# MattAgostini/ECE1782-Smith-Waterman-CUDA

Measured on AMD Instinct MI355X. Metric: GCUPS (DP cell updates/s) query-vs-SwissProt, 1/2/4/8 MI355X; bit-exact scores, higher is better.
Workload: dtype fp16

## Files before the change

ece1782-smith-waterman-cuda_amd/capi.py:

```python
import ctypes
import os
import weakref

import numpy as np

PKG_DIR = os.path.dirname(os.path.abspath(__file__))
LIB_DIR = os.path.join(PKG_DIR, "lib")
LIB_PATH = os.environ.get("SW_AMD_LIB") or os.path.join(LIB_DIR, "libswamd.so")

SW_OK = 0
SW_ALPHABET = 25
MATRIX_BLOSUM50_REF = 0
MATRIX_BLOSUM62 = 1
MATRIX_IDENTITY3 = 2
MATRIX_BLOSUM50_CHAR = 3

EXPORTED = (
    "sw_version", "sw_build_id", "sw_last_error", "sw_encode", "sw_builtin_matrix",
    "sw_create", "sw_destroy", "sw_stream", "sw_set_stream",
    "sw_opts_init", "sw_opts_from_env", "sw_set_opts", "sw_get_opts",
    "sw_db_create", "sw_db_free", "sw_db_get_stats", "sw_db_set_long_threshold", "sw_db_reset_adaptive",
    "sw_scan", "sw_scan_device", "sw_scan_batch", "sw_scan_batch_device", "sw_get_timing",
    "sw_timing_reset", "sw_timing_total", "sw_stream_wait_scan", "sw_last_kernel", "sw_last_intra_kernel",
    "sw_topk", "sw_topk_device", "sw_topk_keys_device", "sw_topk_device_ids", "sw_scan_topk",
    "sw_scan_rank_device", "sw_score_pair",
    "sw_align",
    "sw_pssm_create", "sw_pssm_free", "sw_pssm_length", "sw_scan_pssm", "sw_scan_pssm_device",
    "sw_scan_pssm_topk", "sw_align_pssm",
    "sw_db_save", "sw_db_load", "sw_db_subjects", "sw_db_create_synthetic", "sw_synth_tables",
    "sw_synth_lengths", "sw_group_create", "sw_group_destroy", "sw_group_info", "sw_group_handle",
    "sw_group_db_create", "sw_group_db_free", "sw_group_db_shard", "sw_group_scan", "sw_group_topk",
)


class SWError(RuntimeError):
    pass


class Scoring(ctypes.Structure):
    _fields_ = [("matrix", ctypes.POINTER(ctypes.c_int8)),
                ("gap_open", ctypes.c_int32),
                ("gap_extend", ctypes.c_int32)]


class DbStats(ctypes.Structure):
    _fields_ = [("n_subjects", ctypes.c_int64), ("residues", ctypes.c_int64),
                ("packed_cells", ctypes.c_int64), ("n_blocks", ctypes.c_int64),
                ("n_long", ctypes.c_int64), ("device_bytes", ctypes.c_int64),
                ("max_length", ctypes.c_int32), ("long_threshold", ctypes.c_int32),
                ("coop_blocks", ctypes.c_int32), ("coop_residues", ctypes.c_int64),
                ("max_id", ctypes.c_int32), ("pair_blocks", ctypes.c_int32),
                ("pair_merged", ctypes.c_int32), ("pair_residues", ctypes.c_int64)]


class Alignment(ctypes.Structure):
    _fields_ = [("score", ctypes.c_int32), ("q_begin", ctypes.c_int32), ("q_end", ctypes.c_int32),
                ("s_begin", ctypes.c_int32), ("s_end", ctypes.c_int32), ("ops_len", ctypes.c_int32)]


class Opts(ctypes.Structure):
    INT_FIELDS = ("lpt", "lpt_pipe", "quad_width", "pair_width", "pair_group", "coop_width", "coop_skew",
                  "intra_x2", "intra_x2_rows", "intra_i16_first", "inter_i16_span", "int16_guard",
                  "rescue_stats", "tail_pairs", "lpt_persist", "lpt_rows", "tri_width", "lpt_pipe_tail", "drain_spin")
    _fields_ = [("size", ctypes.c_int32)] + [(f, ctypes.c_int32) for f in INT_FIELDS] + \
        [("inter_variant", ctypes.c_char * 16), ("trace_file", ctypes.c_char * 256)]

    def as_dict(self):
        d = {f: getattr(self, f) for f in self.INT_FIELDS}
        d["inter_variant"] = self.inter_variant.decode()
        d["trace_file"] = self.trace_file.decode()
        return d


def opts_from_env():
    o = Opts()
    _check(lib().sw_opts_from_env(ctypes.byref(o)))
    return o


class Timing(ctypes.Structure):
    _fields_ = [("inter_ms", ctypes.c_float), ("intra_ms", ctypes.c_float),
                ("total_ms", ctypes.c_float), ("rescued", ctypes.c_int32),
                ("launches", ctypes.c_int32), ("coop_ms", ctypes.c_float),
                ("wave_ms", ctypes.c_float)]


_LIB = None


def lib():
    global _LIB
    if _LIB is not None:
        return _LIB
    if not os.path.exists(LIB_PATH):
        raise SWError("HIP library %s not built; run __graft_entry__.build() "
                      "or make -C ece1782-smith-waterman-cuda_amd/csrc" % LIB_PATH)
    try:
        import torch
    except ImportError:
        pass
    L = ctypes.CDLL(LIB_PATH)
    vp, i32, i64 = ctypes.c_void_p, ctypes.c_int32, ctypes.c_int64
    u8p = ctypes.POINTER(ctypes.c_uint8)
    i32p = ctypes.POINTER(ctypes.c_int32)
    i64p = ctypes.POINTER(ctypes.c_int64)
    sig = {
        "sw_version": (i32, []),
        "sw_build_id": (ctypes.c_char_p, []),
        "sw_last_error": (ctypes.c_char_p, []),
        "sw_encode": (ctypes.c_int, [ctypes.c_char_p, i64, u8p]),
        "sw_builtin_matrix": (ctypes.c_int, [i32, ctypes.POINTER(ctypes.c_int8)]),
        "sw_create": (ctypes.c_int, [i32, ctypes.POINTER(vp)]),
        "sw_destroy": (ctypes.c_int, [vp]),
        "sw_stream": (vp, [vp]),
        "sw_set_stream": (ctypes.c_int, [vp, vp]),
        "sw_opts_init": (ctypes.c_int, [ctypes.POINTER(Opts)]),
        "sw_opts_from_env": (ctypes.c_int, [ctypes.POINTER(Opts)]),
        "sw_set_opts": (ctypes.c_int, [vp, ctypes.POINTER(Opts)]),
        "sw_get_opts": (ctypes.c_int, [vp, ctypes.POINTER(Opts)]),
        "sw_db_reset_adaptive": (ctypes.c_int, [vp]),
        "sw_db_create": (ctypes.c_int, [vp, u8p, i64p, i64, i32p, ctypes.POINTER(vp)]),
        "sw_db_free": (ctypes.c_int, [vp]),
        "sw_db_get_stats": (ctypes.c_int, [vp, ctypes.POINTER(DbStats)]),
        "sw_db_set_long_threshold": (ctypes.c_int, [vp, i32]),
        "sw_scan": (ctypes.c_int, [vp, vp, u8p, i32, ctypes.POINTER(Scoring), i32p]),
        "sw_scan_device": (ctypes.c_int, [vp, vp, u8p, i32, ctypes.POINTER(Scoring), vp]),
        "sw_scan_batch": (ctypes.c_int, [vp, vp, u8p, i64p, i32, ctypes.POINTER(Scoring), i32p]),
        "sw_scan_batch_device": (ctypes.c_int, [vp, vp, u8p, i64p, i32, ctypes.POINTER(Scoring), vp]),
        "sw_get_timing": (ctypes.c_int, [vp, ctypes.POINTER(Timing)]),
        "sw_timing_reset": (ctypes.c_int, [vp]),
        "sw_timing_total": (ctypes.c_int, [vp, ctypes.POINTER(Timing), i32p]),
        "sw_stream_wait_scan": (ctypes.c_int, [vp, vp]),
        "sw_last_kernel": (ctypes.c_char_p, [vp]),
        "sw_last_intra_kernel": (ctypes.c_char_p, [vp]),
        "sw_db_save": (ctypes.c_int, [vp, ctypes.c_char_p]),
        "sw_db_create_synthetic": (ctypes.c_int, [vp, ctypes.c_uint64, i64, i64, ctypes.POINTER(vp)]),
        "sw_synth_tables": (ctypes.c_int, [i32p, u8p]),
        "sw_synth_lengths": (ctypes.c_int, [ctypes.c_uint64, i64, i64, i32p]),
        "sw_db_subjects": (ctypes.c_int, [vp, i64p, i32p]),
        "sw_db_load": (ctypes.c_int, [vp, ctypes.c_char_p, ctypes.POINTER(vp)]),
        "sw_align": (ctypes.c_int, [vp, vp, u8p, i32, ctypes.POINTER(Scoring), i32p, i32,
                                    ctypes.POINTER(Alignment), ctypes.c_char_p, ctypes.c_int64]),
        "sw_pssm_create": (ctypes.c_int, [vp, ctypes.POINTER(ctypes.c_int8), i32, ctypes.POINTER(vp)]),
        "sw_pssm_free": (ctypes.c_int, [vp]),
        "sw_pssm_length": (ctypes.c_int, [vp, i32p]),
        "sw_scan_pssm": (ctypes.c_int, [vp, vp, vp, i32, i32, i32p]),
        "sw_scan_pssm_device": (ctypes.c_int, [vp, vp, vp, i32, i32, vp]),
        "sw_scan_pssm_topk": (ctypes.c_int, [vp, vp, vp, i32, i32, i32, i64p]),
        "sw_align_pssm": (ctypes.c_int, [vp, vp, vp, i32, i32, i32p, i32,
                                         ctypes.POINTER(Alignment), ctypes.c_char_p, ctypes.c_int64]),
        "sw_topk": (ctypes.c_int, [i32p, i64, i32, i32p, i32p]),
        "sw_topk_device": (ctypes.c_int, [vp, vp, i64, i64, i32, vp]),
        "sw_topk_keys_device": (ctypes.c_int, [vp, vp, i64, i32, vp]),
        "sw_topk_device_ids": (ctypes.c_int, [vp, vp, i64, vp, i32, vp]),
        "sw_scan_topk": (ctypes.c_int, [vp, vp, u8p, i32, ctypes.POINTER(Scoring), i32, i64p]),
        "sw_scan_rank_device": (ctypes.c_int, [vp, vp, u8p, i32, ctypes.POINTER(Scoring), vp, i32, vp, i64, vp]),
        "sw_score_pair": (ctypes.c_int, [vp, u8p, i32, u8p, i32, ctypes.POINTER(Scoring), i32p]),
        "sw_group_create": (ctypes.c_int, [i32p, i32, ctypes.POINTER(vp)]),
        "sw_group_destroy": (ctypes.c_int, [vp]),
        "sw_group_info": (ctypes.c_char_p, [vp]),
        "sw_group_handle": (ctypes.c_int, [vp, i32, ctypes.POINTER(vp)]),
        "sw_group_db_create": (ctypes.c_int, [vp, u8p, i64p, i64, i32p, ctypes.POINTER(vp)]),
        "sw_group_db_free": (ctypes.c_int, [vp]),
        "sw_group_db_shard": (ctypes.c_int, [vp, i32, i64p, i64p]),
        "sw_group_scan": (ctypes.c_int, [vp, vp, u8p, i32, ctypes.POINTER(Scoring), i32p]),
        "sw_group_topk": (ctypes.c_int, [vp, vp, u8p, i32, ctypes.POINTER(Scoring), i32, i64p]),
    }
    for name, (res, args) in sig.items():
        fn = getattr(L, name)
        fn.restype = res
        fn.argtypes = args
    built, want = L.sw_build_id().decode(), source_id()
    if built != want:
        raise SWError("stale HIP library %s: built from sources %s, the tree's are %s; rebuild it "
                      "(__graft_entry__.build() or make -C ece1782-smith-waterman-cuda_amd/csrc)"
                      % (LIB_PATH, built, want))
    _LIB = L
    return L


def source_id(repo_root=None):
    import importlib.util
    spec = importlib.util.spec_from_file_location("_sw_build_id", os.path.join(PKG_DIR, "csrc", "build_id.py"))
    mod = importlib.util.module_from_spec(spec)
    spec.loader.exec_module(mod)
    return mod.source_id(repo_root or os.path.dirname(PKG_DIR))


def build_id():
    return lib().sw_build_id().decode()


def _check(rc):
    if rc != SW_OK:
        raise SWError("sw_amd error %d: %s" % (rc, lib().sw_last_error().decode(errors="replace")))


def _u8(a):
    a = np.ascontiguousarray(a, dtype=np.uint8)
    return a, a.ctypes.data_as(ctypes.POINTER(ctypes.c_uint8))


def encode(seq):
    b = seq.encode() if isinstance(seq, str) else bytes(seq)
    out = np.empty(len(b), dtype=np.uint8)
    _check(lib().sw_encode(b, len(b), out.ctypes.data_as(ctypes.POINTER(ctypes.c_uint8))))
    return out


def builtin_matrix(mid=MATRIX_BLOSUM50_REF):
    out = np.empty(625, dtype=np.int8)
    _check(lib().sw_builtin_matrix(mid, out.ctypes.data_as(ctypes.POINTER(ctypes.c_int8))))
    return out.reshape(25, 25)


class _ScoringArg:

    def __init__(self, matrix=None, gap_open=2, gap_extend=None):
        gap_extend = gap_open if gap_extend is None else gap_extend
        if matrix is None:
            self._m = None
            self.s = Scoring(None, gap_open, gap_extend)
        else:
            self._m = np.ascontiguousarray(np.asarray(matrix, dtype=np.int8).reshape(625))
            self.s = Scoring(self._m.ctypes.data_as(ctypes.POINTER(ctypes.c_int8)), gap_open, gap_extend)

    def ptr(self):
        return ctypes.byref(self.s)


class Handle:

    def __init__(self, device=0, env_opts=True):
        h = ctypes.c_void_p()
        _check(lib().sw_create(device, ctypes.byref(h)))
        self._h = h
        self.device = device
        self._dbs = weakref.WeakSet()
        if env_opts:
            _check(lib().sw_set_opts(h, ctypes.byref(opts_from_env())))

    def get_opts(self):
        o = Opts()
        _check(lib().sw_get_opts(self._h, ctypes.byref(o)))
        return o

    def set_opts(self, opts=None, **fields):
        o = Opts()
        if opts is None:
            o = self.get_opts()
        else:
            ctypes.memmove(ctypes.byref(o), ctypes.byref(opts), ctypes.sizeof(Opts))
        for k, v in fields.items():
            if k in ("inter_variant", "trace_file"):
                setattr(o, k, (v or "").encode())
            elif k in Opts.INT_FIELDS:
                setattr(o, k, -1 if v is None else int(v))
            else:
                raise TypeError("unknown sw_opts field %r" % k)
        _check(lib().sw_set_opts(self._h, ctypes.byref(o)))

    def reset_opts(self):
        o = Opts()
        _check(lib().sw_opts_init(ctypes.byref(o)))
        _check(lib().sw_set_opts(self._h, ctypes.byref(o)))

    @property
    def ptr(self):
        return self._h

    def close(self):
        if self._h:
            for db in list(self._dbs):
                db.close()
            lib().sw_destroy(self._h)
            self._h = None

    def __del__(self):
        try:
            self.close()
        except Exception:
            pass

    def stream(self):
        return lib().sw_stream(self._h)

    def set_stream(self, hip_stream):
        _check(lib().sw_set_stream(self._h, hip_stream))

    def timing(self):
        t = Timing()
        _check(lib().sw_get_timing(self._h, ctypes.byref(t)))
        return {k: getattr(t, k) for k, _ in Timing._fields_}

    def timing_reset(self):
        _check(lib().sw_timing_reset(self._h))

    def stream_wait_scan(self, hip_stream):
        _check(lib().sw_stream_wait_scan(self._h, hip_stream))

    def last_kernel(self):
        return lib().sw_last_kernel(self._h).decode()

    def last_intra_kernel(self):
        return lib().sw_last_intra_kernel(self._h).decode()

    def timing_total(self):
        t = Timing()
        n = ctypes.c_int32()
        _check(lib().sw_timing_total(self._h, ctypes.byref(t), ctypes.byref(n)))
        out = {k: getattr(t, k) for k, _ in Timing._fields_ if k != "rescued"}
        out["scans"] = n.value
        return out

    def topk_device(self, scores_dev_ptr, n, k, keys_out_dev_ptr, id_base=0):
        _check(lib().sw_topk_device(self._h, ctypes.c_void_p(scores_dev_ptr), n, id_base, k,
                                    ctypes.c_void_p(keys_out_dev_ptr)))

    def topk_device_ids(self, scores_dev_ptr, n, ids_dev_ptr, k, keys_out_dev_ptr):
        _check(lib().sw_topk_device_ids(self._h, ctypes.c_void_p(scores_dev_ptr), n, ctypes.c_void_p(ids_dev_ptr),
                                        k, ctypes.c_void_p(keys_out_dev_ptr)))

    def topk_keys_device(self, keys_dev_ptr, n, k, keys_out_dev_ptr):
        _check(lib().sw_topk_keys_device(self._h, ctypes.c_void_p(keys_dev_ptr), n, k,
                                         ctypes.c_void_p(keys_out_dev_ptr)))

    def score_pair(self, query_codes, subject_codes, matrix=None, gap_open=2, gap_extend=None):
        q, qp = _u8(query_codes)
        s, sp = _u8(subject_codes)
        sc = _ScoringArg(matrix, gap_open, gap_extend)
        out = ctypes.c_int32()
        _check(lib().sw_score_pair(self._h, qp, len(q), sp, len(s), sc.ptr(), ctypes.byref(out)))
        return out.value


class Pssm:

    def __init__(self, handle, rows):
        self.handle = handle
        r = np.asarray(rows)
        if r.size and (r.ndim != 2 or r.shape[1] != SW_ALPHABET):
            raise SWError("a PSSM is a [qlen][%d] table" % SW_ALPHABET)
        if r.size and (r.min() < -128 or r.max() > 127):
            raise SWError("sw_amd error -1: PSSM entries must be in -100..100")
        r = np.ascontiguousarray(r, dtype=np.int8).reshape(-1, SW_ALPHABET)
        p = ctypes.c_void_p()
        _check(lib().sw_pssm_create(handle.ptr, r.ctypes.data_as(ctypes.POINTER(ctypes.c_int8)), len(r),
                                    ctypes.byref(p)))
        self._p = p
        handle._dbs.add(self)

    @property
    def ptr(self):
        return self._p

    def __len__(self):
        n = ctypes.c_int32()
        _check(lib().sw_pssm_length(self._p, ctypes.byref(n)))
        return n.value

    def close(self):
        if self._p:
            if self.handle.ptr:
                lib().sw_pssm_free(self._p)
            self._p = None

    def __del__(self):
        try:
            self.close()
        except Exception:
            pass


class Database:

    def __init__(self, handle, residues, offsets, ids=None, long_threshold=None):
        self.handle = handle
        r, rp = _u8(residues)
        o = np.ascontiguousarray(offsets, dtype=np.int64)
        n = len(o) - 1
        idp = None
        if ids is not None:
            self._ids = np.ascontiguousarray(ids, dtype=np.int32)
            idp = self._ids.ctypes.data_as(ctypes.POINTER(ctypes.c_int32))
            self.n_out = int(self._ids.max()) + 1 if n > 0 else 0
        else:
            self.n_out = n
        d = ctypes.c_void_p()
        _check(lib().sw_db_create(handle.ptr, rp, o.ctypes.data_as(ctypes.POINTER(ctypes.c_int64)),
                                  n, idp, ctypes.byref(d)))
        self._d = d
        self.n = n
        handle._dbs.add(self)
        if long_threshold is not None:
            self.set_long_threshold(long_threshold)

    @classmethod
    def synthetic(cls, handle, seed, n, id_base=0, long_threshold=None):
        self = cls.__new__(cls)
        self.handle = handle
        d = ctypes.c_void_p()
        _check(lib().sw_db_create_synthetic(handle.ptr, seed, id_base, n, ctypes.byref(d)))
        self._d = d
        self.n = n
        self.n_out = n
        handle._dbs.add(self)
        if long_threshold is not None:
            self.set_long_threshold(long_threshold)
        return self
# ... 265 lines not shown
```

ece1782-smith-waterman-cuda_amd/csrc/sw_capi.cpp:

```cpp
#include <algorithm>
#include <cmath>
#include <atomic>
#include <cstdio>
#include <cstdlib>
#include <cstring>
#include <memory>
#include <new>
#include <numeric>
#include <string>
#include <thread>
#include <unordered_map>
#include <vector>

#include "sw_host.h"
#include "sw_plan.h"

using swk::DevPtr;
using swk::Event;
using swk::HostPtr;
using swk::Stream;

namespace {

thread_local std::string g_err;

constexpr int kF16Span = 2048;

uint32_t f16_pair(int v) {
    const _Float16 x = static_cast<_Float16>(static_cast<float>(v));
    uint16_t b;
    std::memcpy(&b, &x, 2);
    return static_cast<uint32_t>(b) | (static_cast<uint32_t>(b) << 16);
}

int fail(int code, const std::string& msg) {
    g_err = msg;
    return code;
}

#define MARK(k, s)                                  \
    do {                                            \
        HIPCHECK(hipEventRecord(h->ev[k].get(), (s)));    \
        *h->ev_rec |= 1u << (k);                    \
    } while (0)

const int8_t kBlosum50Ref[625] = {
    5, -2, -1, -2, -1, -1, -1, 0, -2, -1, -2, -1, -1, -3, -1, 1, 0, -3, -2, 0, -2, -2, -1, -1, 0,
    -2, 7, -1, -2, -4, 1, 0, -3, 0, -4, -3, 3, -2, -3, -3, -1, -1, -3, -1, -3, -1, -3, 0, -1, 0,
    -1, -1, 7, 2, -2, 0, 0, 0, 1, -3, -4, 0, -2, -4, -2, 1, 0, -4, -2, -3, 5, -4, 0, -1, 0,
    -2, -2, 2, 8, -4, 0, 2, -1, -1, -4, -4, -1, -4, -5, -1, 0, -1, -5, -3, -4, 6, -4, 1, -1, 0,
    -1, -4, -2, -4, 13, -3, -3, -3, -3, -2, -2, -3, -2, -2, -4, -1, -1, -5, -3, -1, -3, -2, -3, -1, 0,
    -1, 1, 0, 0, -3, 7, 2, -2, 1, -3, -2, 2, 0, -4, -1, 0, -1, -1, -1, -3, 0, -3, 4, -1, 0,
    -1, 0, 0, 2, -3, 2, 6, -3, 0, -4, -3, 1, -2, -3, -1, -1, -1, -3, -2, -3, 1, -3, 5, -1, 0,
    0, -3, 0, -1, -3, -2, -3, 8, -2, -4, -4, -2, -3, -4, -2, 0, -2, -3, -3, -4, -1, -4, -2, -1, 0,
    -2, 0, 1, -1, -3, 1, 0, -2, 10, -4, -3, 0, -1, -1, -2, -1, -2, -3, 2, -4, 0, -3, 0, -1, 0,
    -1, -4, -3, -4, -2, -3, -4, -4, -4, 5, 2, -3, 2, 0, -3, -3, -1, -3, -1, 4, -4, 4, -3, -1, 0,
    -2, -3, -4, -4, -2, -2, -3, -4, -3, 2, 5, -3, 3, 1, -4, -3, -1, -2, -1, 1, -4, 4, -3, -1, 0,
    -1, 3, 0, -1, -3, 2, 1, -2, 0, -3, -3, 6, -2, -4, -1, 0, -1, -3, -2, -3, 0, -3, 1, -1, 0,
    -1, -2, -2, -4, -2, 0, -2, -3, -1, 2, 3, -2, 7, 0, -3, -2, -1, -1, 0, 1, -3, 2, -1, -1, 0,
    -3, -3, -4, -5, -2, -4, -3, -4, -1, 0, 1, -4, 0, 8, -4, -3, -2, 1, 4, -1, -4, 1, -4, -1, 0,
    -1, -3, -2, -1, -4, -1, -1, -2, -2, -3, -4, -1, -3, -4, 10, -1, -1, -4, -3, -3, -2, -3, -1, -1, 0,
    1, -1, 1, 0, -1, 0, -1, 0, -1, -3, -3, 0, -2, -3, -1, 5, 2, -4, -2, -2, 0, -3, 0, -1, 0,
    0, -1, 0, -1, -1, -1, -1, -2, -2, -1, -1, -1, -1, -2, -1, 2, 5, -3, -2, 0, 0, -1, -1, -1, 0,
    -3, -3, -4, -5, -5, -1, -3, -3, -3, -3, -2, -3, -1, 1, -4, -4, -3, 15, 2, -3, -5, -2, -2, -1, 0,
    -2, -1, -2, -3, -3, -1, -2, -3, 2, -1, -1, -2, 0, 4, -3, -2, -2, 2, 8, -1, -3, -1, -2, -1, 0,
    0, -3, -3, -4, -1, -3, -3, -4, -4, 4, 1, -3, 1, -1, -3, -2, 0, -3, -1, 5, -3, 2, -3, -1, 0,
    -2, -1, 5, 6, -3, 0, 1, -1, 0, -4, -4, 0, -3, -4, -2, 0, 0, -5, -3, -3, 6, -4, 1, -1, 0,
    -2, -3, -4, -4, -2, -3, -3, -4, -3, 4, 4, -3, 2, 1, -3, -3, -1, -2, -1, 2, -4, 4, -3, -1, 0,
    -1, 0, 0, 1, -3, 4, 5, -2, 0, -3, -3, 1, -1, -4, -1, 0, -1, -2, -2, -3, 1, -3, 5, -1, 0,
    -1, -1, -1, -1, -1, -1, -1, -1, -1, -1, -1, -1, -1, -1, -1, -1, -1, -1, -1, -1, -1, -1, -1, -1, 0,
    0, 0, 0, 0, 0, 0, 0, 0, 0, 0, 0, 0, 0, 0, 0, 0, 0, 0, 0, 0, 0, 0, 0, 0, 0,
};

const int8_t kBlosum62[625] = {
    4, -1, -2, -2, 0, -1, -1, 0, -2, -1, -1, -1, -1, -2, -1, 1, 0, -3, -2, 0, -2, -1, -1, 0, -4,
    -1, 5, 0, -2, -3, 1, 0, -2, 0, -3, -2, 2, -1, -3, -2, -1, -1, -3, -2, -3, -1, -2, 0, -1, -4,
    -2, 0, 6, 1, -3, 0, 0, 0, 1, -3, -3, 0, -2, -3, -2, 1, 0, -4, -2, -3, 3, -3, 0, -1, -4,
    -2, -2, 1, 6, -3, 0, 2, -1, -1, -3, -4, -1, -3, -3, -1, 0, -1, -4, -3, -3, 4, -3, 1, -1, -4,
    0, -3, -3, -3, 9, -3, -4, -3, -3, -1, -1, -3, -1, -2, -3, -1, -1, -2, -2, -1, -3, -1, -3, -2, -4,
    -1, 1, 0, 0, -3, 5, 2, -2, 0, -3, -2, 1, 0, -3, -1, 0, -1, -2, -1, -2, 0, -2, 3, -1, -4,
    -1, 0, 0, 2, -4, 2, 5, -2, 0, -3, -3, 1, -2, -3, -1, 0, -1, -3, -2, -2, 1, -3, 4, -1, -4,
    0, -2, 0, -1, -3, -2, -2, 6, -2, -4, -4, -2, -3, -3, -2, 0, -2, -2, -3, -3, -1, -4, -2, -1, -4,
    -2, 0, 1, -1, -3, 0, 0, -2, 8, -3, -3, -1, -2, -1, -2, -1, -2, -2, 2, -3, 0, -3, 0, -1, -4,
    -1, -3, -3, -3, -1, -3, -3, -4, -3, 4, 2, -3, 1, 0, -3, -2, -1, -3, -1, 3, -3, 3, -3, -1, -4,
    -1, -2, -3, -4, -1, -2, -3, -4, -3, 2, 4, -2, 2, 0, -3, -2, -1, -2, -1, 1, -4, 3, -3, -1, -4,
    -1, 2, 0, -1, -3, 1, 1, -2, -1, -3, -2, 5, -1, -3, -1, 0, -1, -3, -2, -2, 0, -3, 1, -1, -4,
    -1, -1, -2, -3, -1, 0, -2, -3, -2, 1, 2, -1, 5, 0, -2, -1, -1, -1, -1, 1, -3, 2, -1, -1, -4,
    -2, -3, -3, -3, -2, -3, -3, -3, -1, 0, 0, -3, 0, 6, -4, -2, -2, 1, 3, -1, -3, 0, -3, -1, -4,
    -1, -2, -2, -1, -3, -1, -1, -2, -2, -3, -3, -1, -2, -4, 7, -1, -1, -4, -3, -2, -2, -3, -1, -2, -4,
    1, -1, 1, 0, -1, 0, 0, 0, -1, -2, -2, 0, -1, -2, -1, 4, 1, -3, -2, -2, 0, -2, 0, 0, -4,
    0, -1, 0, -1, -1, -1, -1, -2, -2, -1, -1, -1, -1, -2, -1, 1, 5, -2, -2, 0, -1, -1, -1, 0, -4,
    -3, -3, -4, -4, -2, -2, -3, -2, -2, -3, -2, -3, -1, 1, -4, -3, -2, 11, 2, -3, -4, -2, -3, -2, -4,
    -2, -2, -2, -3, -2, -1, -2, -3, 2, -1, -1, -2, -1, 3, -3, -2, -2, 2, 7, -1, -3, -1, -2, -1, -4,
    0, -3, -3, -3, -1, -2, -2, -3, -3, 3, 1, -2, 1, -1, -2, -2, 0, -3, -1, 4, -3, 2, -2, -1, -4,
    -2, -1, 3, 4, -3, 0, 1, -1, 0, -3, -4, 0, -3, -3, -2, 0, -1, -4, -3, -3, 4, -3, 1, -1, -4,
    -1, -2, -3, -3, -1, -2, -3, -4, -3, 3, 3, -3, 2, 0, -3, -2, -1, -2, -1, 2, -3, 3, -3, -1, -4,
    -1, 0, 0, 1, -3, 3, 4, -2, 0, -3, -3, 1, -1, -3, -1, 0, -1, -3, -2, -2, 1, -3, 4, -1, -4,
    0, -1, -1, -1, -2, -1, -1, -1, -1, -1, -1, -1, -1, -1, -2, 0, 0, -2, -1, -1, -1, -1, -1, -1, -4,
    -4, -4, -4, -4, -4, -4, -4, -4, -4, -4, -4, -4, -4, -4, -4, -4, -4, -4, -4, -4, -4, -4, -4, -4, 1,
};

int8_t g_encode_lut[256];
bool g_lut_ready = false;

void init_lut() {
    if (g_lut_ready) return;
    static const char letters[] = "ARNDCQEGHILKMFPSTWYVBJZX";
    for (int c = 0; c < 256; ++c) g_encode_lut[c] = SW_CODE_STAR;
    for (int k = 0; k < 24; ++k) g_encode_lut[static_cast<unsigned char>(letters[k])] = static_cast<int8_t>(k);
    g_lut_ready = true;
}

int64_t round_up(int64_t v, int64_t m) { return (v + m - 1) / m * m; }

int default_threads() {
    unsigned n = std::thread::hardware_concurrency();
    if (n == 0) n = 4;
    return static_cast<int>(std::min(16u, n));
}

template <class F>
void parallel_for(int64_t n, F&& f, int64_t grain = 64) {
    const int nt = static_cast<int>(std::min<int64_t>(default_threads(), std::max<int64_t>(1, n / grain)));
    if (nt <= 1) {
        for (int64_t i = 0; i < n; ++i) f(i);
        return;
    }
    std::atomic<int64_t> next{0};
    std::vector<std::thread> th;
    for (int t = 0; t < nt; ++t)
        th.emplace_back([&] {
            for (;;) {
                const int64_t i0 = next.fetch_add(grain);
                if (i0 >= n) break;
                const int64_t i1 = std::min(n, i0 + grain);
                for (int64_t i = i0; i < i1; ++i) f(i);
            }
        });
    for (auto& t : th) t.join();
}

template <class T>
struct NoInitAlloc : std::allocator<T> {
    template <class U>
    struct rebind {
        using other = NoInitAlloc<U>;
    };
    NoInitAlloc() = default;
    template <class U>
    NoInitAlloc(const NoInitAlloc<U>&) {}
    template <class U, class... A>
    void construct(U* p, A&&... a) {
        if constexpr (sizeof...(A) == 0) ::new (static_cast<void*>(p)) U;
        else ::new (static_cast<void*>(p)) U(std::forward<A>(a)...);
    }
};

std::vector<int64_t> length_order(const std::vector<int64_t>& offs, int64_t n) {
    std::vector<int64_t> order(n);
    int64_t maxl = 0;
    for (int64_t k = 0; k < n; ++k) maxl = std::max(maxl, offs[k + 1] - offs[k]);
    if (maxl > (int64_t(1) << 22)) {
        std::iota(order.begin(), order.end(), 0);
        std::stable_sort(order.begin(), order.end(), [&](int64_t x, int64_t y) {
            return offs[x + 1] - offs[x] > offs[y + 1] - offs[y];
        });
        return order;
    }
    std::vector<int64_t> start(static_cast<size_t>(maxl) + 2, 0);
    for (int64_t k = 0; k < n; ++k) ++start[static_cast<size_t>(maxl - (offs[k + 1] - offs[k]) + 1)];
    for (size_t l = 1; l < start.size(); ++l) start[l] += start[l - 1];
    for (int64_t k = 0; k < n; ++k) order[start[static_cast<size_t>(maxl - (offs[k + 1] - offs[k]))]++] = k;
    return order;
}

}

int swk::set_error(int code, const std::string& msg) { return fail(code, msg); }

struct ScanEvents {
    Event ev[8];
    unsigned rec = 0;
    int launches = 0;
    bool merged = false;
};

namespace {
sw_opts default_opts() {
    sw_opts o;
    std::memset(&o, 0, sizeof o);
    o.size = static_cast<int32_t>(sizeof o);
    for (int32_t* f : {&o.lpt, &o.lpt_pipe, &o.quad_width, &o.pair_width, &o.pair_group, &o.coop_width,
                       &o.coop_skew, &o.intra_x2, &o.intra_x2_rows, &o.intra_i16_first, &o.inter_i16_span,
                       &o.int16_guard, &o.rescue_stats, &o.tail_pairs, &o.lpt_persist, &o.lpt_rows,
                       &o.tri_width, &o.lpt_pipe_tail, &o.drain_spin})
        *f = -1;
    return o;
}
}

struct sw_handle {
    int device = 0;
    int cus = 0;
    Stream stream;
    bool own_stream = false;
    ~sw_handle() { if (!own_stream) stream.release(); }
    std::vector<ScanEvents> evpool;
    size_t nscans = 0;
    Event* ev = nullptr;
    unsigned* ev_rec = nullptr;
    Stream side;
    Stream side2;
    Stream tail;
    Event main_done, side_done;
    Event tail_done[2];
    bool tail_pending[2] = {};
    int parity = 0;
    Event coop_done;
    Event fork2;
    struct ProfSlot {
        DevPtr<int8_t> d;
        size_t dcap = 0;
        hipEvent_t last_end = nullptr;
        bool pending = false;
        Event tail_read;
        bool tail_pending = false;
    };
    HostPtr<uint8_t> stage[2];
    size_t stage_cap = 0;
    Event stage_ev[2];
    bool stage_pending[2] = {};
    static constexpr int kProfSlots = 4;
    ProfSlot prof[kProfSlots];
    int prof_next = 0;
    DevPtr<int32_t> d_scores;
    size_t scores_cap = 0;
    DevPtr<int64_t> d_topk_work;
    std::string last_kernel = "none";
    std::string last_intra = "none";
    size_t topk_cap = 0;
    bool timed = false;
    bool had_intra = false;
    int launches = 0;
    HostPtr<int32_t> h_fault;
    int32_t* d_fault = nullptr;
    int open_slot = -1;
    sw_opts opts = default_opts();
};

static std::atomic<uint64_t> g_fault_epoch{0};

static int check_fault(sw_handle* h) {
    if (h && h->h_fault.get() && __atomic_load_n(h->h_fault.get(), __ATOMIC_ACQUIRE)) {
        __atomic_store_n(h->h_fault.get(), 0, __ATOMIC_RELEASE);
        g_fault_epoch.fetch_add(1);
        return fail(SW_E_DEVICE, "sw_scan_lpt: a claimed rescue-list entry never appeared; the handle's scans "
                                 "since the last successful call may hold unrescued scores");
    }
    return SW_OK;
}

static hipError_t quiesce(sw_handle* h) {
    hipError_t first = hipSuccess;
    for (hipStream_t st : {h->stream.get(), h->side.get(), h->side2.get(), h->tail.get()})
        if (st) {
            const hipError_t e = hipStreamSynchronize(st);
            if (first == hipSuccess) first = e;
        }
    return first;
}

struct Readback {
    struct Obs {
        uint64_t key = 0, qhash = 0;
        int32_t qlen = 0, nr = 0;
        bool operator==(const Obs& o) const { return key == o.key && qhash == o.qhash && qlen == o.qlen && nr == o.nr; }
    };
    HostPtr<int32_t> host;
    Event ev;
    bool pending = false;
    bool seen = false;
    Obs sent, last;
};

namespace {
int readback_record(Readback& r, const Readback::Obs& o, const int32_t* w0, const int32_t* w1, hipStream_t s) {
    if (r.pending || (r.seen && r.last == o)) return SW_OK;
    if (!r.host.get()) {
        HostPtr<int32_t> host;
        Event ev;
        HIPCHECK(swk::host_alloc(host, 2 * sizeof(int32_t), hipHostMallocDefault));
        HIPCHECK(swk::event_create(ev, hipEventDisableTiming));
        r.host = std::move(host);
        r.ev = std::move(ev);
    }
    HIPCHECK(hipMemcpyAsync(r.host.get(), w0, sizeof(int32_t), hipMemcpyDeviceToHost, s));
    if (w1) HIPCHECK(hipMemcpyAsync(r.host.get() + 1, w1, sizeof(int32_t), hipMemcpyDeviceToHost, s));
    HIPCHECK(hipEventRecord(r.ev.get(), s));
    r.pending = true;
    r.sent = o;
    return SW_OK;
}

bool readback_take(Readback& r) {
    if (!r.pending || hipEventQuery(r.ev.get()) != hipSuccess) return false;
    r.pending = false;
    r.seen = true;
    r.last = r.sent;
    return true;
}

void readback_reset(Readback& r) { r.pending = r.seen = false; }

}

struct sw_db {
    sw_handle* h = nullptr;
    int64_t n = 0;
    int64_t residues = 0;
    int32_t max_len = 0;
    int32_t max_id = -1;
    int32_t long_threshold = 0;
    struct LptTable {
        int32_t qpad, rows , qpad_intra, ri, npair, group , tail , n;
        bool affine;
        bool tri;
        int32_t npipe;
        int32_t pipe_opt;
        int32_t pipe_tail;
        int32_t tail_opt;
        DevPtr<int32_t> d_order;
        std::vector<float> cost;
    };
    static constexpr int kDrainSlots = 32;
    struct Layout {
        DevPtr<uint8_t> d_res;
        DevPtr<uint64_t> d_blk_off;
        DevPtr<uint32_t> d_blk_groups;
        DevPtr<uint32_t> d_blk_cols;
        DevPtr<int32_t> d_lane_ids;
        DevPtr<int32_t> d_ids;
        DevPtr<int32_t> d_bnd_h, d_bnd_f;
        DevPtr<int32_t> d_rescue;
        DevPtr<int32_t> d_lrescue;
        DevPtr<int32_t> d_rbnd_h, d_rbnd_f, d_rlbnd_h, d_rlbnd_f;
        bool rbnd_tried = false;
        DevPtr<uint8_t> d_lres;
        DevPtr<uint64_t> d_loff;
// ... 692 lines not shown
    h->ev_rec = &h->evpool[h->nscans].rec;
    *h->ev_rec = 0;
    h->evpool[h->nscans].launches = 0;
    h->evpool[h->nscans].merged = false;
    ++h->nscans;
    return SW_OK;
}

int rank_after(sw_handle* h, sw_db* db, const int32_t* scores_dev, const RankReq& rq) {
    swk::TopkSrc src;
    int rc;
    if ((rc = rank_src(db, scores_dev, rq, &src))) return rc;
    if ((rc = ensure_topk_work(h, swk::topk_workspace_bytes(db->n, rq.k)))) return rc;
    HIPCHECK(swk::launch_topk(src, db->n, rq.k, rq.out, h->d_topk_work.get(), h->stream.get()));
    ++h->launches;
    return SW_OK;
}

struct BndRows {
    int32_t *h, *f, *lh, *lf;
};
BndRows pass_rows(const sw_db::Layout& l) { return {l.d_bnd_h.get(), l.d_bnd_f.get(), l.d_lbnd_h.get(), l.d_lbnd_f.get()}; }
BndRows tail_rows(const sw_db::Layout& l) { return {l.d_rbnd_h.get(), l.d_rbnd_f.get(), l.d_rlbnd_h.get(), l.d_rlbnd_f.get()}; }

struct Scan {
    sw_handle* h = nullptr;
    sw_db* db = nullptr;
    swplan::ScanPlan plan;
    swplan::PlanScoring sc;
    int32_t qlen = 0;
    uint64_t skey = 0, qhash = 0;
    int32_t* scores = nullptr;
    int par = 0;
    int32_t *listA = nullptr, *listB = nullptr, *maxA = nullptr, *headA = nullptr;
    int32_t *list1 = nullptr, *list2 = nullptr, *head1 = nullptr;
    int32_t* lpt_next = nullptr;
    bool deferred = false;
    Profiles P;
    swk::InterArgs a{};
    swk::IntraArgs ia{}, x{};
    bool inter_tail = false, intra_tail = false;
};

int scan_empty(sw_handle* h, sw_db* db, int32_t* scores_dev, bool defer, const RankReq* rq) {
    int rc;
    db->last_ncoop = 0;
    db->last_npair = 0;
    h->last_kernel = "none";
    h->last_intra = "none";
    if (!defer && (rc = join_tails(h))) return rc;
    MARK(0, h->stream.get());
    if (db->max_id >= 0) HIPCHECK(hipMemsetAsync(scores_dev, 0, static_cast<size_t>(db->max_id + 1) * 4, h->stream.get()));
    if (rq && (rc = rank_after(h, db, scores_dev, *rq))) return rc;
    for (int k = 1; k < 8; ++k) MARK(k, h->stream.get());
    h->timed = true;
    return SW_OK;
}

int scan_lists(Scan& c, bool defer) {
    sw_handle* h = c.h;
    sw_db* db = c.db;
    const swplan::ScanPlan& p = c.plan;
    int rc;
    const int64_t rstride = 2 * (db->nblocks + 1) + 4;
    const int64_t lstride = 2 * (db->nlong + 1) + 2;
    if (p.rescue && db->nblocks && !db->lay.d_rescue.get()) {
        HIPCHECK(swk::dev_alloc(db->lay.d_rescue, 2 * rstride * sizeof(int32_t)));
        HIPCHECK(hipMemsetAsync(db->lay.d_rescue.get(), 0xff, 2 * rstride * sizeof(int32_t), h->stream.get()));
        db->lay.device_bytes += 2 * rstride * sizeof(int32_t);
    }
    if ((p.multi_inter || p.multi_intra) && (rc = ensure_bnd(db, p.affine, p.intra_x2))) return rc;
    if (p.intra_x2 && !db->lay.d_lrescue.get()) {
        HIPCHECK(swk::dev_alloc(db->lay.d_lrescue, 2 * lstride * sizeof(int32_t)));
        HIPCHECK(hipMemsetAsync(db->lay.d_lrescue.get(), 0xff, 2 * lstride * sizeof(int32_t), h->stream.get()));
        db->lay.device_bytes += 2 * lstride * sizeof(int32_t);
    }
    if (db->list_epoch != g_fault_epoch.load()) {
        if ((rc = join_tails(h))) return rc;
        hipStream_t const s = h->stream.get();
        if (int32_t* l = db->lay.d_rescue.get()) HIPCHECK(hipMemsetAsync(l, 0xff, 2 * rstride * sizeof(int32_t), s));
        if (int32_t* l = db->lay.d_lrescue.get()) HIPCHECK(hipMemsetAsync(l, 0xff, 2 * lstride * sizeof(int32_t), s));
        db->list_epoch = g_fault_epoch.load();
    }
    c.par = h->parity;
    h->parity ^= 1;
    if (h->tail_pending[c.par]) {
        HIPCHECK(hipStreamWaitEvent(h->stream.get(), h->tail_done[c.par].get(), 0));
        h->tail_pending[c.par] = false;
    }
    if (p.drain && (rc = join_tails(h))) return rc;
    if (db->lay.d_rescue.get()) {
        c.listA = db->lay.d_rescue.get() + c.par * rstride;
        c.listB = c.listA + db->nblocks + 1;
        c.maxA = c.listA + 2 * (db->nblocks + 1);
        c.headA = c.maxA + 2;
        if (p.lpt && h->opts.lpt_persist != 0) c.lpt_next = c.maxA + 1;
    }
    if (db->lay.d_lrescue.get()) {
        c.list1 = db->lay.d_lrescue.get() + c.par * lstride;
        c.list2 = c.list1 + db->nlong + 1;
        c.head1 = c.list2 + db->nlong + 1;
    }
    c.deferred = !p.drain && defer && (!(p.multi_inter || p.multi_intra) || ensure_rbnd(db, p.affine, p.intra_x2));
    return SW_OK;
}

int scan_profiles(Scan& c, const QuerySrc& src, const int8_t* mat) {
    const swplan::ScanPlan& p = c.plan;
    const bool d = p.drain;
    int32_t* const cA = (p.rescue && c.db->nblocks) ? c.listA : nullptr;
    int32_t* const c1 = p.intra_x2 ? c.list1 : nullptr;
    int32_t* const reset[10] = {cA, (cA && p.f16) ? c.listB : nullptr, (cA && p.f16) ? c.maxA : nullptr, c1,
                                c1 ? c.list2 : nullptr, d ? c.headA : nullptr, d ? c.headA + 1 : nullptr,
                                d ? c.head1 : nullptr, d ? c.head1 + 1 : nullptr, c.lpt_next};
    const int rc = build_profiles(c.h, src, mat, c.sc.go, p.affine,
                                  std::max({p.qpad_inter, p.qpad_rescue, p.qpad_coop, p.qpad_list, p.qpad_intra2}),
                                  p.shape.x2s || p.intra_x2, p.ri, p.qpad_intra, reset, &c.P);
    c.h->evpool[c.h->nscans - 1].merged = p.lpt;
    return rc;
}

int inter_args(Scan& c) {
    sw_db* db = c.db;
    const swplan::ScanPlan& p = c.plan;
    const int go = c.sc.go, ge = c.sc.ge;
    swk::InterArgs& a = c.a;
    a.residues = db->lay.d_res.get();
    a.blk_off = db->lay.d_blk_off.get();
    a.blk_groups = db->lay.d_blk_groups.get();
    a.blk_cols = db->lay.d_blk_cols.get();
    a.lane_ids = db->lay.d_lane_ids.get();
    a.nblocks = static_cast<int32_t>(db->nblocks);
    a.prof = c.P.dev + (p.shape.x2s ? c.P.off16 : c.P.off8);
    a.prof_stride = c.P.stride;
    a.qpad = p.qpad_inter;
    a.gap_open = go;
    a.gap_extend = ge;
    a.bnd_h = db->lay.d_bnd_h.get();
    a.bnd_f = db->lay.d_bnd_f.get();
    a.scores = c.scores;
    if (c.h->opts.trace_file[0]) {
        if (!db->lay.h_trace.get()) {
            db->lay.trace_entries = static_cast<size_t>(2 * db->nblocks + db->nlong + 8);
            HIPCHECK(swk::host_alloc(db->lay.h_trace, 32 * db->lay.trace_entries, hipHostMallocMapped));
            std::memset(db->lay.h_trace.get(), 0, 32 * db->lay.trace_entries);
        }
        HIPCHECK(hipHostGetDevicePointer(reinterpret_cast<void**>(&a.trace), db->lay.h_trace.get(), 0));
    }
    if (p.rescue) {
        a.rescue_count = c.listA;
        a.rescue_list = c.listA + 1;
        if (p.f16) a.rescue_max = c.maxA;
        const int zero = -kF16Span + 2 * ge;
        a.sat_limit = kF16Span - zero - 2 * std::max(c.sc.max_s, 1) - 26 * ge;
        for (int j = 0; j < 32; ++j) a.f16_step[j] = f16_pair(j * ge + zero);
        a.f16_gog = f16_pair(go - ge);
        a.f16_zero = f16_pair(zero);
        a.f16_diff[0] = f16_pair(4 * ge);
        a.f16_diff[1] = f16_pair(8 * ge);
        a.f16_diff[2] = f16_pair(16 * ge);
    }
    a.re_last = p.re_last;
    if (p.lpt) {
        a.blk_first = p.npair;
        a.blk_quad = p.nquad;
        a.blk_tri = p.ntri ? 1 : 0;
        a.blk_tail = static_cast<int32_t>(db->nblocks) - p.ntail;
    } else if (p.npair) {
        a.blk_base = p.nr;
        a.blk_first = std::max(p.npair, p.nr);
    } else {
        a.blk_first = p.ncoop;
    }
    return SW_OK;
}

void intra_args(Scan& c) {
    const sw_db* db = c.db;
    swk::IntraArgs& ia = c.ia;
    ia.residues = db->lay.d_lres.get();
    ia.subj_off = db->lay.d_loff.get();
    ia.subj_len = db->lay.d_llen.get();
    ia.subj_id = db->lay.d_lid.get();
    ia.nsubj = static_cast<int32_t>(db->nlong);
    ia.prof = c.P.dev + c.P.intra_off;
    ia.qpad = c.plan.qpad_intra;
    ia.gap_open = c.sc.go;
    ia.gap_extend = c.sc.ge;
    ia.bnd_h = db->lay.d_lbnd_h.get();
    ia.bnd_f = db->lay.d_lbnd_f.get();
    ia.scores = c.scores;
}

void intra_x2_args(Scan& c) {
    const swplan::ScanPlan& p = c.plan;
    const int go = c.sc.go, ge = c.sc.ge;
    swk::IntraArgs& x = c.x;
    x = c.ia;
    x.prof = c.P.dev + c.P.off16;
    x.prof_stride = c.P.stride;
    x.bias = p.affine ? 0 : go;
    x.qpad = p.qpad_intra2;
    const int zero = -kF16Span + 2 * ge;
    x.sat_limit = kF16Span - zero - 2 * std::max(c.sc.max_s, 1) - swk::intra_bias_rows(p.ri2) * ge;
    for (int j = 0; j < swk::kIntraSteps; ++j) x.f16_step[j] = f16_pair(j * ge + zero);
    x.f16_zero = f16_pair(zero);
    x.f16_gog = f16_pair(go - ge);
    int32_t* const flagged = p.intra_i16_first ? c.list2 : c.list1;
    x.rescue_count = flagged;
    x.rescue_list = flagged + 1;
}

int scan_args(Scan& c) {
    if (c.db->nlong) {
        intra_args(c);
        if (c.plan.intra_x2) intra_x2_args(c);
    }
    return c.db->nblocks ? inter_args(c) : SW_OK;
}

struct RescueStages {
    swk::InterArgs a16, a32;
    swk::IntraArgs i16, i32;
};
RescueStages rescue_stages(const Scan& c, const swk::IntraArgs& x, const BndRows& r, bool in_launch) {
    const swplan::ScanPlan& p = c.plan;
    auto items = [](int32_t* list) { return list ? list + 1 : nullptr; };
    int32_t* const l32 = p.f16 ? c.listB : c.listA;
    RescueStages s{c.a, c.a, x, c.ia};
    s.a16.bnd_h = s.a32.bnd_h = r.h;
    s.a16.bnd_f = s.a32.bnd_f = r.f;
    s.a16.qpad = p.qpad_list;
    s.a16.re_last = p.affine ? 32 : 48;
    s.a32.re_last = swplan::rescue_rows(p.affine);
    s.a16.rescue_list = items(c.listB);
    s.a16.rescue_count = c.listB;
    s.a16.rescue_max = nullptr;
    s.a32.prof = c.P.dev + c.P.off8;
    s.a32.qpad = p.qpad_rescue;
    s.a32.rescue_list = nullptr;
    s.a32.rescue_count = nullptr;
    s.i16.bnd_h = s.i32.bnd_h = r.lh;
    s.i16.bnd_f = s.i32.bnd_f = r.lf;
    s.i16.rescue_list = items(c.list2);
    s.i16.rescue_count = c.list2;
    if (in_launch) {
        s.a16.trace = s.a32.trace = nullptr;
        s.a32.rescue_max = nullptr;
    } else {
        s.a16.blk_list = items(c.listA);
        s.a16.blk_count = c.listA;
        s.a32.blk_list = items(l32);
        s.a32.blk_count = l32;
        s.i16.subj_list = items(c.list1);
        s.i16.list_count = c.list1;
        s.i32.subj_list = items(c.list2);
        s.i32.list_count = c.list2;
    }
    return s;
}

int launch_inter_tail(Scan& c, hipStream_t st, const RescueStages& s) {
    if (c.plan.f16) {
        HIPCHECK(swk::launch_inter_x2s_list(s.a16, c.plan.affine, st));
        ++c.h->launches;
    }
    HIPCHECK(swk::launch_inter_rescue(s.a32, c.plan.affine, st));
    ++c.h->launches;
    return SW_OK;
}

int launch_intra_tail(Scan& c, hipStream_t st, const RescueStages& s) {
    if (!c.plan.intra_i16_first) {
        HIPCHECK(swk::launch_intra_x2_list16(s.i16, c.plan.ri2, st));
        ++c.h->launches;
    }
    HIPCHECK(swk::launch_intra(s.i32, c.plan.ri, c.plan.affine, st));
    ++c.h->launches;
    return SW_OK;
}

int intra_tail(Scan& c, hipStream_t is) {
    c.intra_tail = true;
    if (c.deferred) {
        HIPCHECK(hipEventRecord(c.h->side_done.get(), is));
        return SW_OK;
    }
    return launch_intra_tail(c, is, rescue_stages(c, c.x, pass_rows(c.db->lay), false));
}

int inter_tail(Scan& c) {
    sw_handle* h = c.h;
    const swplan::ScanPlan& p = c.plan;
    int rc;
    if (p.f16 && p.rescue &&
        (rc = readback_record(c.db->icount, {c.skey, c.qhash, c.qlen, p.nr}, c.listA, c.maxA, h->stream.get())))
        return rc;
    c.inter_tail = p.rescue && !p.drain;
    if (!c.inter_tail) return SW_OK;
    if (c.deferred) {
        HIPCHECK(hipEventRecord(h->main_done.get(), h->stream.get()));
        return SW_OK;
    }
    return launch_inter_tail(c, h->stream.get(), rescue_stages(c, c.x, pass_rows(c.db->lay), false));
}

int long_pass(Scan& c) {
// ... 282 lines not shown
    HIPCHECK(hipMemcpyAsync(scores_host, h->d_scores.get(), n * 4, hipMemcpyDeviceToHost, h->stream.get()));
    HIPCHECK(hipStreamSynchronize(h->stream.get()));
    return check_fault(h);
}

int scan_topk_host(sw_handle* h, const sw_db* cdb, const QuerySrc& src, int32_t k, int64_t* keys_host) {
    sw_db* db = const_cast<sw_db*>(cdb);
    if (!h || !db || !keys_host || k <= 0 || k > 4096) return fail(SW_E_INVALID, "bad argument (1 <= k <= 4096)");
    if (db->n == 0) {
        for (int32_t i = 0; i < k; ++i) keys_host[i] = INT64_MIN;
        return SW_OK;
    }
    int rc;
    HIPCHECK(hipSetDevice(h->device));
    const size_t slots = static_cast<size_t>(db->max_id + 1);
    if ((rc = ensure_scores(h, slots + static_cast<size_t>(2 * k) + 2))) return rc;
    int64_t* keys_dev = reinterpret_cast<int64_t*>(h->d_scores.get() + round_up(static_cast<int64_t>(slots), 2));
    const RankReq rq{k, nullptr, 0, keys_dev};
    if ((rc = scan_impl(h, db, src, h->d_scores.get(), false, &rq))) return rc;
    HIPCHECK(hipMemcpyAsync(keys_host, keys_dev, static_cast<size_t>(k) * sizeof(int64_t), hipMemcpyDeviceToHost,
                            h->stream.get()));
    HIPCHECK(hipStreamSynchronize(h->stream.get()));
    return check_fault(h);
}

}

namespace {
int topk_impl(sw_handle* h, const int32_t* scores, const int64_t* keys, int64_t n, int64_t id_base,
              const int32_t* ids, int32_t k, int64_t* out) {
    if (!h || !out || n < 0 || k <= 0 || k > 4096 || (n > 0 && !scores && !keys))
        return fail(SW_E_INVALID, "bad top-k arguments (1 <= k <= 4096)");
    if (id_base < 0 || id_base + n > (int64_t(1) << 31)) return fail(SW_E_INVALID, "ids must fit in 31 bits");
    HIPCHECK(hipSetDevice(h->device));
    int rc;
    if ((rc = check_fault(h))) return rc;
    if ((rc = ensure_topk_work(h, swk::topk_workspace_bytes(n, k)))) return rc;
    swk::TopkSrc src{};
    src.scores = keys ? nullptr : scores;
    src.keys = keys;
    src.gid = ids;
    src.id_base = id_base;
    HIPCHECK(swk::launch_topk(src, n, k, out, h->d_topk_work.get(), h->stream.get()));
    return SW_OK;
}
}

extern "C" {

int32_t sw_version(void) { return 10000 * 0 + 100 * 2 + 0; }

#ifndef SW_SOURCE_ID
#define SW_SOURCE_ID "unknown"
#endif
const char* sw_build_id(void) { return SW_SOURCE_ID; }

const char* sw_last_error(void) { return g_err.c_str(); }

int sw_encode(const char* ascii, int64_t n, uint8_t* codes) {
    if ((!ascii || !codes) && n > 0) return fail(SW_E_INVALID, "null argument");
    init_lut();
    for (int64_t i = 0; i < n; ++i) codes[i] = static_cast<uint8_t>(g_encode_lut[static_cast<unsigned char>(ascii[i])]);
    return SW_OK;
}

int sw_builtin_matrix(int32_t id, int8_t* out625) {
    if (!out625) return fail(SW_E_INVALID, "null argument");
    if (id == SW_MATRIX_BLOSUM50_REF) {
        std::memcpy(out625, kBlosum50Ref, 625);
    } else if (id == SW_MATRIX_BLOSUM62) {
        std::memcpy(out625, kBlosum62, 625);
    } else if (id == SW_MATRIX_IDENTITY3) {
        for (int a = 0; a < 25; ++a)
            for (int b = 0; b < 25; ++b) out625[a * 25 + b] = static_cast<int8_t>(a == b ? 3 : -3);
    } else if (id == SW_MATRIX_BLOSUM50_CHAR) {
        std::memcpy(out625, kBlosum50Ref, 625);
        for (int k = 0; k < 25; ++k) out625[SW_CODE_STAR * 25 + k] = out625[k * 25 + SW_CODE_STAR] = -5;
        out625[SW_CODE_STAR * 25 + SW_CODE_STAR] = 1;
    } else {
        return fail(SW_E_INVALID, "unknown matrix id");
    }
    return SW_OK;
}

int sw_create(int32_t device, sw_handle** out) {
    if (!out) return fail(SW_E_INVALID, "null argument");
    *out = nullptr;
    int ndev = 0;
    if (hipGetDeviceCount(&ndev) != hipSuccess || ndev == 0) return fail(SW_E_NODEVICE, "no HIP device visible");
    if (device < 0 || device >= ndev) return fail(SW_E_INVALID, "device index out of range");
    HIPCHECK(hipSetDevice(device));
    std::unique_ptr<sw_handle> h(new (std::nothrow) sw_handle());
    if (!h) return fail(SW_E_NOMEM, "out of host memory");
    h->device = device;
    if (hipDeviceGetAttribute(&h->cus, hipDeviceAttributeMultiprocessorCount, device) != hipSuccess) h->cus = 0;
    HIPCHECK(swk::stream_create(h->stream, hipStreamNonBlocking));
    h->own_stream = true;
    HIPCHECK(swk::stream_create(h->side, hipStreamNonBlocking));
    HIPCHECK(swk::stream_create(h->side2, hipStreamNonBlocking));
    int least = 0, greatest = 0;
    HIPCHECK(hipDeviceGetStreamPriorityRange(&least, &greatest));
    HIPCHECK(swk::stream_create(h->tail, hipStreamNonBlocking, greatest));
    for (Event* ev : {&h->main_done, &h->side_done, &h->tail_done[0], &h->tail_done[1], &h->coop_done, &h->fork2,
                      &h->stage_ev[0], &h->stage_ev[1]})
        HIPCHECK(swk::event_create(*ev, hipEventDisableTiming));
    for (auto& S : h->prof) HIPCHECK(swk::event_create(S.tail_read, hipEventDisableTiming));
    HIPCHECK(swk::host_alloc(h->h_fault, sizeof(int32_t), hipHostMallocMapped));
    *h->h_fault.get() = 0;
    HIPCHECK(hipHostGetDevicePointer(reinterpret_cast<void**>(&h->d_fault), h->h_fault.get(), 0));
    *out = h.release();
    return SW_OK;
}

int sw_destroy(sw_handle* h) {
    if (!h) return SW_OK;
    (void)hipSetDevice(h->device);
    (void)quiesce(h);
    delete h;
    return SW_OK;
}

void* sw_stream(sw_handle* h) { return h ? reinterpret_cast<void*>(h->stream.get()) : nullptr; }

int sw_opts_init(sw_opts* o) {
    if (!o) return fail(SW_E_INVALID, "null argument");
    *o = default_opts();
    return SW_OK;
}

int sw_opts_from_env(sw_opts* o) {
    int rc;
    if ((rc = sw_opts_init(o))) return rc;
    const struct {
        const char* name;
        int32_t* field;
    } ints[] = {{"SW_LPT", &o->lpt},
                {"SW_LPT_PIPE", &o->lpt_pipe},
                {"SW_QUAD_WIDTH", &o->quad_width},
                {"SW_PAIR_WIDTH", &o->pair_width},
                {"SW_PAIR_GROUP", &o->pair_group},
                {"SW_COOP_WIDTH", &o->coop_width},
                {"SW_COOP_SKEW", &o->coop_skew},
                {"SW_INTRA_X2", &o->intra_x2},
                {"SW_INTRA_X2_RI", &o->intra_x2_rows},
                {"SW_INTRA_I16_FIRST", &o->intra_i16_first},
                {"SW_INTER_I16_SPAN", &o->inter_i16_span},
                {"SW_INT16_GUARD", &o->int16_guard},
                {"SW_RESCUE_STATS", &o->rescue_stats},
                {"SW_TAIL_PAIRS", &o->tail_pairs},
                {"SW_LPT_PERSIST", &o->lpt_persist},
                {"SW_LPT_ROWS", &o->lpt_rows},
                {"SW_TRI_WIDTH", &o->tri_width},
                {"SW_LPT_PIPE_TAIL", &o->lpt_pipe_tail},
                {"SW_DRAIN_SPIN", &o->drain_spin}};
    for (const auto& k : ints)
        if (const char* e = std::getenv(k.name); e && e[0]) *k.field = std::atoi(e);
    if (const char* e = std::getenv("SW_INTER_VARIANT"))
        std::snprintf(o->inter_variant, sizeof o->inter_variant, "%s", e);
    if (const char* e = std::getenv("SW_TRACE_FILE")) std::snprintf(o->trace_file, sizeof o->trace_file, "%s", e);
    return SW_OK;
}

int sw_set_opts(sw_handle* h, const sw_opts* o) {
    if (!h || !o) return fail(SW_E_INVALID, "null argument");
    if (o->size != static_cast<int32_t>(sizeof(sw_opts)))
        return fail(SW_E_INVALID, "sw_opts.size mismatch (initialise with sw_opts_init)");
    if (o->pair_group != -1 && o->pair_group != 2 && o->pair_group != 4)
        return fail(SW_E_INVALID, "sw_opts.pair_group must be -1, 2 or 4");
    h->opts = *o;
    h->opts.inter_variant[sizeof h->opts.inter_variant - 1] = 0;
    h->opts.trace_file[sizeof h->opts.trace_file - 1] = 0;
    return SW_OK;
}

int sw_get_opts(const sw_handle* h, sw_opts* o) {
    if (!h || !o) return fail(SW_E_INVALID, "null argument");
    *o = h->opts;
    return SW_OK;
}

int sw_set_stream(sw_handle* h, void* hip_stream) {
    if (!h) return fail(SW_E_INVALID, "null handle");
    HIPCHECK(hipStreamSynchronize(h->stream.get()));
    if (!h->own_stream) h->stream.release();
    h->own_stream = false;
    if (hip_stream) {
        h->stream = Stream(reinterpret_cast<hipStream_t>(hip_stream));
    } else {
        HIPCHECK(swk::stream_create(h->stream, hipStreamNonBlocking));
        h->own_stream = true;
    }
    return SW_OK;
}

int sw_db_create(sw_handle* h, const uint8_t* residues, const int64_t* offsets, int64_t n, const int32_t* ids,
                 sw_db** out) {
    if (!h || !out || n < 0 || (n > 0 && !offsets)) return fail(SW_E_INVALID, "null argument");
    *out = nullptr;
    if (n > 0 && offsets[0] != 0) return fail(SW_E_INVALID, "offsets[0] must be 0");
    for (int64_t k = 0; k < n; ++k)
        if (offsets[k + 1] < offsets[k]) return fail(SW_E_INVALID, "offsets must be non-decreasing");
    const int64_t total = n > 0 ? offsets[n] : 0;
    if (total > 0 && !residues) return fail(SW_E_INVALID, "null residues");
    for (int64_t k = 0; k < n; ++k)
        if (offsets[k + 1] - offsets[k] > (int64_t(1) << 30)) return fail(SW_E_INVALID, "subject too long");
    std::unique_ptr<sw_db> db(new (std::nothrow) sw_db());
    if (!db) return fail(SW_E_NOMEM, "out of host memory");
    db->h = h;
    db->n = n;
    try {
        db->h_residues.resize(static_cast<size_t>(total));
        db->h_offsets.assign(offsets, offsets + n + 1);
        if (n == 0) db->h_offsets.assign(1, 0);
        db->h_ids.resize(n);
        for (int64_t k = 0; k < n; ++k) db->h_ids[k] = ids ? ids[k] : static_cast<int32_t>(k);
    } catch (...) {
        return fail(SW_E_NOMEM, "out of host memory");
    }
    constexpr int64_t kPiece = int64_t(1) << 20;
    std::atomic<bool> bad{false};
    parallel_for((total + kPiece - 1) / kPiece, [&](int64_t c) {
        const int64_t lo = c * kPiece, hi = std::min(total, lo + kPiece);
        std::memcpy(db->h_residues.data() + lo, residues + lo, static_cast<size_t>(hi - lo));
        uint8_t m = 0;
        for (int64_t k = lo; k < hi; ++k) m = std::max(m, residues[k]);
        if (m >= SW_ALPHABET) bad = true;
    }, 1);
    if (bad) return fail(SW_E_INVALID, "residue code out of range (use sw_encode)");
    db->residues = total;
    for (int64_t k = 0; k < n; ++k) {
        db->max_len = std::max<int32_t>(db->max_len, static_cast<int32_t>(offsets[k + 1] - offsets[k]));
        if (db->h_ids[k] < 0) return fail(SW_E_INVALID, "ids must be >= 0");
        db->max_id = std::max(db->max_id, db->h_ids[k]);
    }
    db->long_threshold = swplan::default_long_threshold(plan_view(db.get()));
    HIPCHECK(hipSetDevice(h->device));
    if (int rc = build_db(db.get())) return rc;
    *out = db.release();
    return SW_OK;
}

namespace {
constexpr char kDbMagic[8] = {'S', 'W', 'A', 'M', 'D', 'D', 'B', '1'};
struct DbFileHeader {
    char magic[8];
    int64_t n;
    int64_t residues;
    int32_t max_len;
    int32_t version;
    uint64_t fnv;
};

uint64_t fnv1a(uint64_t h, const void* p, size_t n) {
    const auto* b = static_cast<const uint8_t*>(p);
    for (size_t k = 0; k < n; ++k) h = (h ^ b[k]) * 1099511628211ull;
    return h;
}
}

int sw_db_save(const sw_db* db, const char* path) {
    if (!db || !path) return fail(SW_E_INVALID, "null argument");
    const int64_t n = db->n;
    const std::vector<int64_t> order = length_order(db->h_offsets, n);
    auto len = [&](int64_t k) { return db->h_offsets[k + 1] - db->h_offsets[k]; };
    std::vector<int64_t> offs(n + 1, 0);
    std::vector<int32_t> ids(n);
    std::vector<uint8_t> res(static_cast<size_t>(db->residues));
    for (int64_t k = 0; k < n; ++k) {
        const int64_t src = order[k];
        subject_residues(db, src, res.data() + offs[k]);
        offs[k + 1] = offs[k] + len(src);
        ids[k] = db->h_ids[src];
    }
    DbFileHeader hd{};
    std::memcpy(hd.magic, kDbMagic, 8);
    hd.n = n;
    hd.residues = db->residues;
    hd.max_len = db->max_len;
    hd.version = 1;
    uint64_t f = 1469598103934665603ull;
    f = fnv1a(f, offs.data(), offs.size() * sizeof(int64_t));
    f = fnv1a(f, ids.data(), ids.size() * sizeof(int32_t));
    hd.fnv = fnv1a(f, res.data(), res.size());
    FILE* fp = std::fopen(path, "wb");
    if (!fp) return fail(SW_E_IO, std::string("cannot open ") + path);
    bool ok = std::fwrite(&hd, sizeof hd, 1, fp) == 1 &&
              std::fwrite(offs.data(), sizeof(int64_t), offs.size(), fp) == offs.size() &&
              (n == 0 || std::fwrite(ids.data(), sizeof(int32_t), ids.size(), fp) == ids.size()) &&
              (res.empty() || std::fwrite(res.data(), 1, res.size(), fp) == res.size());
    ok = (std::fclose(fp) == 0) && ok;
    if (!ok) return fail(SW_E_IO, std::string("write failed: ") + path);
    return SW_OK;
}

int sw_db_load(sw_handle* h, const char* path, sw_db** out) {
    if (!h || !path || !out) return fail(SW_E_INVALID, "null argument");
    *out = nullptr;
    FILE* fp = std::fopen(path, "rb");
    if (!fp) return fail(SW_E_IO, std::string("cannot open ") + path);
    DbFileHeader hd{};
    std::vector<int64_t> offs;
    std::vector<int32_t> ids;
    std::vector<uint8_t> res;
    int rc = SW_OK;
    if (std::fread(&hd, sizeof hd, 1, fp) != 1 || std::memcmp(hd.magic, kDbMagic, 8) != 0 || hd.version != 1 ||
        hd.n < 0 || hd.residues < 0 || hd.n > (int64_t(1) << 40) || hd.residues > (int64_t(1) << 44)) {
        rc = fail(SW_E_IO, std::string("not a database file (sw_db_save format 1): ") + path);
    } else {
        try {
            offs.resize(hd.n + 1);
            ids.resize(hd.n);
            res.resize(static_cast<size_t>(hd.residues));
// ... 500 lines not shown
```

ece1782-smith-waterman-cuda_amd/csrc/sw_inter_x2.hip:

```cpp
#include <algorithm>

#include "sw_int32.h"
#include "sw_intra_x2.h"
#include "sw_kernels.h"

namespace swk {

typedef short s2 __attribute__((ext_vector_type(2)));
typedef unsigned short u2 __attribute__((ext_vector_type(2)));

__device__ __forceinline__ s2 as_s2(uint32_t x) { return __builtin_bit_cast(s2, x); }
__device__ __forceinline__ uint32_t as_u32(s2 x) { return __builtin_bit_cast(uint32_t, x); }
__device__ __forceinline__ s2 max2(s2 a, s2 b) { return __builtin_elementwise_max(a, b); }
__device__ __forceinline__ s2 usub2(s2 a, u2 g) {
    return __builtin_bit_cast(s2, __builtin_elementwise_sub_sat(__builtin_bit_cast(u2, a), g));
}

__host__ __device__ constexpr int x2_row_dwords(int R) { return (R / 4) % 2 == 1 ? R : R + 4; }

constexpr int kImgCodes = kPadCode + 1;

template <int R>
struct __attribute__((aligned(16))) X2Lds {
    static constexpr int kImg = kImgCodes * x2_row_dwords(R);
// ... 34 lines not shown
__device__ __forceinline__ uint32_t code_of(const uint32_t* w, int jj) { return (w[jj >> 2] >> (8 * (jj & 3))) & 0xffu; }

template <uint32_t RB>
__device__ __forceinline__ uint32_t code_row(const uint32_t* w, int jj, uint32_t base) {
    static_assert(RB < 256, "row stride must fit a byte");
    return __builtin_amdgcn_udot4(w[jj >> 2], RB << (8 * (jj & 3)), base, false);
}

template <int SG>
__device__ __forceinline__ void load_pairs(uint32_t (&v)[SG], const int32_t* p) {
#pragma unroll
    for (int q = 0; q < SG / 4; ++q) {
        const int4 t = *reinterpret_cast<const int4*>(p + 4 * q);
        v[4 * q] = t.x; v[4 * q + 1] = t.y; v[4 * q + 2] = t.z; v[4 * q + 3] = t.w;
    }
}

template <int SG>
__device__ __forceinline__ void store_pairs(int32_t* p, const uint32_t (&v)[SG]) {
#pragma unroll
    for (int q = 0; q < SG / 4; ++q)
        *reinterpret_cast<int4*>(p + 4 * q) = make_int4(v[4 * q], v[4 * q + 1], v[4 * q + 2], v[4 * q + 3]);
}

__device__ __forceinline__ uint32_t lo_lo(uint32_t a, uint32_t b) { return __builtin_amdgcn_perm(b, a, 0x05040100u); }
__device__ __forceinline__ uint32_t hi_lo(uint32_t a, uint32_t b) { return __builtin_amdgcn_perm(b, a, 0x05040302u); }
__device__ __forceinline__ uint32_t hi_hi(uint32_t a, uint32_t b) { return __builtin_amdgcn_perm(b, a, 0x07060302u); }

template <int SG, bool AFFINE>
__device__ __forceinline__ void load_bnd(uint32_t (&v)[SG], const uint32_t* bnd, uint64_t i) {
    if constexpr (AFFINE) {
        load_pairs<SG>(v, reinterpret_cast<const int32_t*>(bnd) + i);
    } else {
        const uint16_t* p = reinterpret_cast<const uint16_t*>(bnd) + i;
        uint32_t w[SG / 2];
        if constexpr (SG == 8) {
            const int4 t = *reinterpret_cast<const int4*>(p);
            w[0] = t.x; w[1] = t.y; w[2] = t.z; w[3] = t.w;
        } else {
            static_assert(SG == 4, "sub-group width");
            const int2 t = *reinterpret_cast<const int2*>(p);
            w[0] = t.x; w[1] = t.y;
        }
#pragma unroll
        for (int q = 0; q < SG; ++q) v[q] = w[q / 2];
    }
}
template <int SG, bool AFFINE>
__device__ __forceinline__ void store_bnd(uint32_t* bnd, uint64_t i, const uint32_t (&hb)[SG]) {
    if constexpr (AFFINE) {
        store_pairs<SG>(reinterpret_cast<int32_t*>(bnd) + i, hb);
    } else {
        uint16_t* p = reinterpret_cast<uint16_t*>(bnd) + i;
        uint32_t w[SG / 2];
#pragma unroll
        for (int q = 0; q < SG / 2; ++q) w[q] = lo_lo(hb[2 * q], hb[2 * q + 1]);
        if constexpr (SG == 8) *reinterpret_cast<int4*>(p) = make_int4(w[0], w[1], w[2], w[3]);
        else *reinterpret_cast<int2*>(p) = make_int2(w[0], w[1]);
    }
}

__device__ __forceinline__ uint32_t to_f16_bits(uint32_t v16) {
    return static_cast<uint32_t>(__builtin_bit_cast(uint16_t, static_cast<_Float16>(static_cast<int16_t>(v16))));
}

template <int R, bool F16>
__device__ __forceinline__ void stage_x2s(X2Lds<R>& L, const int16_t* __restrict__ prof, int stride, int s0,
                                          int lane, int bias, int bias0, int img, int hi0 = R) {
    constexpr int RD = x2_row_dwords(R);
    constexpr int PER = kImgCodes * (R / 8);
    constexpr uint32_t one = F16 ? 0x3c00u : 1u;
    const int n = img < 0 ? 2 * PER : PER;
    for (int t = lane; t < n; t += kLanes) {
        const int im = img < 0 ? t / PER : img;
        const int u = img < 0 ? t % PER : t;
        const int c = u / (R / 8);
        const int k = u % (R / 8);
        const int16_t* src = prof + static_cast<size_t>(c) * stride + s0 + im * hi0 + 8 * k;
        int4 v;
        if (im && (hi0 & 7)) {
            const int2 v0 = *reinterpret_cast<const int2*>(src), v1 = *reinterpret_cast<const int2*>(src + 4);
            v = make_int4(v0.x, v0.y, v1.x, v1.y);
        } else {
            v = *reinterpret_cast<const int4*>(src);
        }
        const uint32_t w[4] = {static_cast<uint32_t>(v.x), static_cast<uint32_t>(v.y), static_cast<uint32_t>(v.z),
                               static_cast<uint32_t>(v.w)};
        uint32_t o[8];
#pragma unroll
        for (int e = 0; e < 4; ++e) {
            const int s0v = static_cast<int16_t>(w[e] & 0xffffu), s1v = static_cast<int16_t>(w[e] >> 16);
            const int b0 = (F16 && k % 2 == 0 && e == 0) ? bias0 : 0;
            uint32_t a0 = static_cast<uint32_t>(s0v) & 0xffffu, a1 = static_cast<uint32_t>(s1v) & 0xffffu;
            if constexpr (F16) {
                a0 = to_f16_bits(static_cast<uint32_t>(s0v + bias + b0));
                a1 = to_f16_bits(static_cast<uint32_t>(s1v + bias));
            }
            o[2 * e] = im ? (a0 << 16) | one : a0 | (one << 16);
            o[2 * e + 1] = im ? (a1 << 16) | one : a1 | (one << 16);
        }
        int4* d = reinterpret_cast<int4*>((im ? L.hi : L.lo) + c * RD + 8 * k);
        d[0] = make_int4(o[0], o[1], o[2], o[3]);
        d[1] = make_int4(o[4], o[5], o[6], o[7]);
    }
}


typedef int v4i __attribute__((ext_vector_type(4)));
typedef __attribute__((address_space(3))) const v4i lds_int4;

__device__ __forceinline__ uint32_t lds_addr(const void* p) {
    return static_cast<uint32_t>(reinterpret_cast<uintptr_t>(p));
}

template <int N>
__device__ __forceinline__ void read_x2a(int4 (&pl)[N], int4 (&ph)[N], uint32_t& aa, uint32_t& ab, int k,
                                         uint32_t dep) {
    asm volatile("" : "+v"(aa), "+v"(ab) : "v"(dep));
    lds_int4* a = reinterpret_cast<lds_int4*>(static_cast<uintptr_t>(aa)) + N * k;
    lds_int4* b = reinterpret_cast<lds_int4*>(static_cast<uintptr_t>(ab)) + N * k;
#pragma unroll
    for (int q = 0; q < N; ++q) {
        pl[q] = __builtin_bit_cast(int4, a[q]);
        ph[q] = __builtin_bit_cast(int4, b[q]);
    }
}

typedef _Float16 h2 __attribute__((ext_vector_type(2)));

template <bool F16>
struct PkCell;

template <>
struct PkCell<false> {
    using V = s2;
    static __device__ __forceinline__ V from(uint32_t x) { return as_s2(x); }
    static __device__ __forceinline__ uint32_t bits(V x) { return as_u32(x); }
};

template <>
struct PkCell<true> {
    using V = h2;
    static __device__ __forceinline__ V from(uint32_t x) { return __builtin_bit_cast(h2, x); }
    static __device__ __forceinline__ uint32_t bits(V x) { return __builtin_bit_cast(uint32_t, x); }
};

__device__ __forceinline__ h2 max3h(h2 a, h2 b, h2 c) {
    return __builtin_elementwise_maximum(__builtin_elementwise_maximum(a, b), c);
}

template <int R, int SG, bool AFFINE, bool F16, int CR = 16, bool SHORT = true>
__device__ __forceinline__ bool x2s_block(const InterArgs& a, int blk, X2Lds<R>& L, int lane);

template <int R, int SG, bool AFFINE, bool F16, bool LIST, int CR = 16>
__global__ __launch_bounds__(256, 2) void sw_inter_x2s(InterArgs a) {
    static_assert(R % CR == 0 && SG % 4 == 0, "shape");
    __shared__ __attribute__((aligned(16))) X2Lds<R> lds[kWavesPerWG];
    const int wave = __builtin_amdgcn_readfirstlane(threadIdx.x >> 6);
    const int lane = threadIdx.x & 63;
    X2Lds<R>& L = lds[wave];
    if constexpr (LIST) {
        const int n = __builtin_amdgcn_readfirstlane(*a.blk_count);
        for (int i = blockIdx.x * kWavesPerWG + wave; i < n; i += gridDim.x * kWavesPerWG)
            x2s_block<R, SG, AFFINE, F16, CR, false>(a, list_take(a.blk_list, i), L, lane);
        return;
    }
    const int blk = a.blk_first + blockIdx.x * kWavesPerWG + wave;
    if (blk >= a.nblocks) return;
    x2s_block<R, SG, AFFINE, F16, CR>(a, blk, L, lane);
}

constexpr int kRowGroup = 16;
constexpr int kAcc = kRowGroup + 8 - 1;
template <bool F16>
struct Best {
    typename PkCell<F16>::V v;
    __device__ __forceinline__ void init(const InterArgs&) { v = PkCell<F16>::from(0u); }
    __device__ __forceinline__ typename PkCell<F16>::V value(const InterArgs&) const { return v; }
};
template <>
struct Best<true> {
    h2 acc[kAcc];
    __device__ __forceinline__ void init(const InterArgs& a) {
#pragma unroll
        for (int k = 0; k < kAcc; ++k) acc[k] = __builtin_bit_cast(h2, a.f16_zero);
    }
    __device__ __forceinline__ void pin() {
        static_assert(kAcc == 23, "pin list");
        asm volatile("" : "+v"(acc[0]), "+v"(acc[1]), "+v"(acc[2]), "+v"(acc[3]), "+v"(acc[4]), "+v"(acc[5]),
                     "+v"(acc[6]), "+v"(acc[7]));
        asm volatile("" : "+v"(acc[8]), "+v"(acc[9]), "+v"(acc[10]), "+v"(acc[11]), "+v"(acc[12]), "+v"(acc[13]),
                     "+v"(acc[14]), "+v"(acc[15]));
        asm volatile("" : "+v"(acc[16]), "+v"(acc[17]), "+v"(acc[18]), "+v"(acc[19]), "+v"(acc[20]),
                     "+v"(acc[21]), "+v"(acc[22]));
    }
    __device__ __forceinline__ h2 value(const InterArgs& a) const {
        const h2 z = __builtin_bit_cast(h2, a.f16_step[0]);
        h2 b = acc[0];
#pragma unroll
        for (int k = 1; k < kAcc; ++k)
            b = __builtin_elementwise_maximum(b, acc[k] - (__builtin_bit_cast(h2, a.f16_step[k]) - z));
        return b;
    }
};

__device__ __forceinline__ uint64_t trace_now() {
#ifdef SW_TRACE_BLOCKS
    return __builtin_amdgcn_s_memrealtime();
#else
    return 0;
#endif
}
__device__ __forceinline__ void trace_block(const InterArgs& a, int blk, uint64_t t0, int lane, uint32_t kind) {
#ifdef SW_TRACE_BLOCKS
    if (a.trace && lane == 0) {
        const uint64_t t1 = __builtin_amdgcn_s_memrealtime();
        const uint32_t hw = __builtin_amdgcn_s_getreg((4) | (0 << 6) | (31 << 11));
        const uint32_t xcc = __builtin_amdgcn_s_getreg((20) | (0 << 6) | (31 << 11));
        uint64_t* t = a.trace + 4 * static_cast<size_t>(blk);
        t[0] = t0;
        t[1] = t1;
        t[2] = hw;
        t[3] = xcc | (static_cast<uint64_t>(kind) << 32);
    }
#else
    (void)a; (void)blk; (void)t0; (void)lane; (void)kind;
#endif
}

template <bool F16>
__device__ __forceinline__ bool x2s_finish(const InterArgs& a, int blk, int lane, typename PkCell<F16>::V best) {
    int b;
    if constexpr (F16)
        b = static_cast<int>(static_cast<float>(__builtin_elementwise_maximum(best.x, best.y))) -
            static_cast<int>(static_cast<float>(__builtin_bit_cast(h2, a.f16_step[0]).x));
    else
        b = max(static_cast<int>(best.x), static_cast<int>(best.y));
    const int id = a.lane_ids[static_cast<size_t>(blk) * kLanes + lane];
    if (id >= 0) a.scores[id] = b;
    if (a.rescue_list) {
        const bool sat = F16 ? (b >= a.sat_limit) : (b >= kSat16 || b < 0);
        const uint64_t m = __builtin_amdgcn_ballot_w64(sat);
        if (m && lane == 0) {
            list_publish(a.rescue_list, a.rescue_count, blk);
            if (a.rescue_max) atomicMax(a.rescue_max, blk);
        }
        return m != 0;
    }
    return false;
}


constexpr int kRingSlots = 4;

template <int SG>
__device__ __forceinline__ void ring_store(int4* ring, int slot, int lane, const uint32_t (&v)[SG]) {
#pragma unroll
    for (int q = 0; q < SG / 4; ++q)
        ring[(slot * (SG / 4) + q) * kLanes + lane] = make_int4(v[4 * q], v[4 * q + 1], v[4 * q + 2], v[4 * q + 3]);
}

template <int SG>
__device__ __forceinline__ void ring_load(uint32_t (&v)[SG], const int4* ring, int slot, int lane) {
#pragma unroll
    for (int q = 0; q < SG / 4; ++q) {
        const int4 t = ring[(slot * (SG / 4) + q) * kLanes + lane];
        v[4 * q] = static_cast<uint32_t>(t.x);
        v[4 * q + 1] = static_cast<uint32_t>(t.y);
        v[4 * q + 2] = static_cast<uint32_t>(t.z);
        v[4 * q + 3] = static_cast<uint32_t>(t.w);
    }
}

template <bool AFFINE>
constexpr bool pair_flags() { return AFFINE; }
struct PairSync {
    int* prog;
    int me;
    int base;
    int pred;
    int pred_base;
    int succ;
    int S;
};
__device__ __forceinline__ void pair_wait(const int* prog, int wave, int need) {
    while (__hip_atomic_load(prog + wave, __ATOMIC_ACQUIRE, __HIP_MEMORY_SCOPE_WORKGROUP) < need)
        __builtin_amdgcn_s_sleep(1);
}

template <int R, int SG, bool AFFINE, bool F16, bool PAIR, int CR = 16, bool CHAIN = false, int RL = R>
__device__ __forceinline__ void x2s_pass(const InterArgs& a, X2Lds<R>& L, uint32_t ncols, uint64_t base, int lane,
                                         int s0, Best<F16>& best, const int4* ring_in, int4* ring_out,
                                         int* tick, const PairSync* ps = nullptr, int chain_passes = 1) {
    static_assert(!(CHAIN && PAIR), "chained passes: single-wave blocks only");
    constexpr int CQ = CR / 4;
    constexpr int NCH = R / CR;
    constexpr int STEPS = SG * NCH;
    using P = PkCell<F16>;
    using V = typename P::V;
    const int16_t* prof16 = reinterpret_cast<const int16_t*>(a.prof);
    const u2 go2 = {static_cast<unsigned short>(a.gap_open), static_cast<unsigned short>(a.gap_open)};
    const u2 ge2 = {static_cast<unsigned short>(a.gap_extend), static_cast<unsigned short>(a.gap_extend)};
    uint32_t* bnd = reinterpret_cast<uint32_t*>(a.bnd_h);
    static_assert(!F16 || (R % kRowGroup == 0 && SG <= 8), "fp16 row groups");
    h2 gog_h = {}, reb_h = {}, grp_h = {};
    if constexpr (F16) {
        gog_h = __builtin_bit_cast(h2, a.f16_gog);
        static_assert(SG == 4 || SG == 8, "rebase constants");
        reb_h = __builtin_bit_cast(h2, a.f16_diff[SG == 4 ? 0 : 1]);
        grp_h = __builtin_bit_cast(h2, a.f16_diff[2]);
    }
    const bool first = (s0 == 0);
    const bool last = (s0 + 2 * R >= a.qpad);
    const uint32_t npass = CHAIN ? static_cast<uint32_t>(chain_passes) : 1u;
    const bool chain_last = CHAIN && static_cast<int>(npass) * 2 * R >= a.qpad;
    const uint32_t total = npass * ncols;
    const int sbias = F16 ? (AFFINE ? 2 : 1) * a.gap_extend : 0;
    const int gbias0 = F16 ? -kRowGroup * a.gap_extend : 0;
    const uint32_t dtop0 = F16 ? a.f16_step[SG - 2 + kRowGroup] : 0u;
    constexpr bool kSh = RL < R;
    if constexpr (kSh) asm volatile("" : "+v"(lane));
    static_assert(!kSh || (RL == R - 4 && !CHAIN), "rows per strip: R, or R - 4 outside a chain");
    static_assert((R - 4 - 1) % kRowGroup == 11, "the short strip's bottom row: 4 ge under the last row's bias");
    h2 dsh_h = {};
    if constexpr (F16) dsh_h = __builtin_bit_cast(h2, a.f16_diff[0]);
    stage_x2s<R, F16>(L, prof16, a.prof_stride, s0, lane, sbias, gbias0, -1, RL);
    __builtin_amdgcn_fence(__ATOMIC_RELEASE, "workgroup");
    __builtin_amdgcn_wave_barrier();
    __builtin_amdgcn_fence(__ATOMIC_ACQUIRE, "workgroup");

    V H[R];
    V E[AFFINE ? R : 1];
#pragma unroll
    for (int r = 0; r < R; ++r) H[r] = P::from(F16 ? a.f16_step[r % kRowGroup + SG - 1] : 0u);
#pragma unroll
    for (int r = 0; r < (AFFINE ? R : 1); ++r) E[r] = P::from(F16 ? a.f16_zero : 0u);
    uint32_t dtop = dtop0;
    uint32_t dl_h[SG], dl_f[SG];
    uint32_t bin[SG], bin_n[SG];
    uint32_t bz[SG];
    uint32_t rc[SG / 4], rp[SG / 4], rn[SG / 4];
#pragma unroll
    for (int q = 0; q < SG; ++q) {
        bz[q] = !F16 ? 0u
                     : AFFINE ? lo_lo(a.f16_step[kRowGroup - 1 + q], a.f16_step[kRowGroup + q])
                              : lo_lo(a.f16_step[kRowGroup - 1 + q], a.f16_step[kRowGroup - 1 + q]);
        dl_h[q] = F16 ? a.f16_step[kRowGroup - 1 + q] : 0u;
        dl_f[q] = F16 ? a.f16_step[kRowGroup + q] : 0u;
        bin[q] = bz[q];
        bin_n[q] = 0;
    }
#pragma unroll
    for (int q = 0; q < SG / 4; ++q) rp[q] = 0x19191919u;
    load_codes<SG>(rc, a.residues + base, true);
    constexpr bool kPairFlags = pair_flags<AFFINE>();
    auto wait_in = [&](uint32_t x) {
        if constexpr (PAIR && kPairFlags)
            pair_wait(ps->prog, ps->pred, ps->pred_base + min(static_cast<int>(x) + 2, ps->S));
    };
    if (!first) {
        wait_in(0);
        if (PAIR && ring_in) ring_load<SG>(bin, ring_in, 0, lane);
        else load_bnd<SG, AFFINE>(bin, bnd, base);
    }
    int4 PL[2][CQ], PH[2][CQ];
    constexpr uint32_t RB = x2_row_dwords(R) * 4;
    const uint32_t blo = lds_addr(L.lo), bhi = lds_addr(L.hi);
    uint32_t aa = code_row<RB>(rc, 0, blo), ab = bhi + kPadCode * RB;
    read_x2a<CQ>(PL[0], PH[0], aa, ab, 0, 0);

    uint32_t lo_p = 0, lo_c = 0;
    bool t2 = false;
    for (uint32_t col0 = 0; col0 <= total; col0 += SG) {
        const bool has_next = col0 + SG <= total;
        const bool next_lo = col0 + SG < total;
        const uint32_t ncol = col0 + SG;
        const bool wrap = CHAIN && lo_c + SG == ncols;
        const uint32_t nreal = CHAIN ? (wrap ? 0u : lo_c + SG) : ncol;
        const bool next_first = CHAIN ? (lo_p == 0 && !wrap) : first;
        const uint64_t noff = (nreal >> 4) * kGroupBytes + (nreal & 15);
        const bool t1 = CHAIN && lo_c == 0 && lo_p > 0 && lo_p < npass;
        const bool next_t1 = CHAIN && wrap && next_lo;
        const bool next_t2 = t1;
        if (t1) {
            stage_x2s<R, F16>(L, prof16, a.prof_stride, static_cast<int>(lo_p) * 2 * R, lane, sbias, gbias0, 0);
#pragma unroll
            for (int r = 0; r < R; ++r) {
                H[r] = P::from(__builtin_amdgcn_perm(P::bits(H[r]), F16 ? a.f16_step[r % kRowGroup + SG - 1] : 0u,
                                                     0x07060100u));
                if constexpr (AFFINE) E[r] = P::from(__builtin_amdgcn_perm(P::bits(E[r]), F16 ? a.f16_zero : 0u, 0x07060100u));
            }
            dtop = __builtin_amdgcn_perm(dtop, dtop0, 0x07060100u);
        }
        if (t2) {
            stage_x2s<R, F16>(L, prof16, a.prof_stride, static_cast<int>(lo_p) * 2 * R, lane, sbias, gbias0, 1);
#pragma unroll
            for (int r = 0; r < R; ++r) {
                H[r] = P::from(__builtin_amdgcn_perm(F16 ? a.f16_step[r % kRowGroup + SG - 1] : 0u, P::bits(H[r]),
                                                     0x07060100u));
                if constexpr (AFFINE) E[r] = P::from(__builtin_amdgcn_perm(F16 ? a.f16_zero : 0u, P::bits(E[r]), 0x07060100u));
            }
            dtop = __builtin_amdgcn_perm(dtop0, dtop, 0x07060100u);
        }
        if (t1 || t2) {
            __builtin_amdgcn_fence(__ATOMIC_RELEASE, "workgroup");
            __builtin_amdgcn_wave_barrier();
            __builtin_amdgcn_fence(__ATOMIC_ACQUIRE, "workgroup");
            aa = code_row<RB>(rc, 0, blo);
            ab = code_row<RB>(rp, 0, bhi);
            read_x2a<CQ>(PL[0], PH[0], aa, ab, 0, 0);
        }
        if (next_t1) {
            __builtin_amdgcn_fence(__ATOMIC_RELEASE, "workgroup");
            __builtin_amdgcn_fence(__ATOMIC_ACQUIRE, "workgroup");
        }
        if (has_next) {
            load_codes<SG>(rn, a.residues + base + noff, next_lo);
            if (!next_first && next_lo) {
                wait_in(ncol / SG);
                if (PAIR && ring_in) ring_load<SG>(bin_n, ring_in, (ncol / SG) % kRingSlots, lane);
                else load_bnd<SG, AFFINE>(bin_n, bnd, base + noff);
            }
        }
        if constexpr (F16) {
#pragma unroll
            for (int r = 0; r < R; ++r) {
                if (r <= RL) H[r] = H[r] - reb_h;
                if constexpr (AFFINE)
                    if (r < RL) E[r] = E[r] - reb_h;
            }
            dtop = P::bits(P::from(dtop) - reb_h);
        }
        auto cell = [&](const int r, const int jj, V& up, V& diag, V& f, const V slo, const V shi) {
            if constexpr (F16 && !AFFINE) {
                const int rg = r % kRowGroup;
                if (rg == 0 && r > 0) up = up - grp_h;
                const h2 t = max3h(H[r], up, __builtin_elementwise_fma(slo, shi, diag));
                const h2 h = __builtin_elementwise_maximum(t, __builtin_bit_cast(h2, a.f16_step[rg + jj]));
                h2& acc = best.acc[rg + jj];
                if (jj & 1) {
                    if (rg + 1 < kRowGroup) acc = max3h(acc, h, H[r + 1]);
                    else acc = __builtin_elementwise_maximum(acc, h);
                } else if (rg == 0) {
                    acc = __builtin_elementwise_maximum(acc, h);
                }
                diag = H[r];
                H[r] = h;
                up = h;
            } else if constexpr (!AFFINE) {
                const s2 h = usub2(max2(max2(H[r], up), slo * shi + diag), go2);
                diag = H[r];
                H[r] = h;
                up = h;
                best.v = max2(best.v, h);
            } else if constexpr (!F16) {
                const s2 h = max2(max2(E[r], f), slo * shi + diag);
                const s2 n = usub2(h, go2);
                E[r] = max2(usub2(E[r], ge2), n);
                f = max2(usub2(f, ge2), n);
                diag = H[r];
                H[r] = h;
                up = h;
                best.v = max2(best.v, h);
            }
        };
        auto cell_d = [&](const int r, const int jj, V& up, V& diag, V& f, const V d) {
          if constexpr (F16 && AFFINE) {
            const int rg = r % kRowGroup;
            if (rg == 0 && r > 0) f = f - grp_h;
            const h2 h = max3h(E[r], f, d);
            const h2 m = h - gog_h;
            E[r] = __builtin_elementwise_maximum(E[r], m);
            f = max3h(f, m, __builtin_bit_cast(h2, a.f16_step[rg + jj + 1]));
            h2& acc = best.acc[rg + jj];
            if (jj & 1) {
                if (rg + 1 < kRowGroup) acc = max3h(acc, h, H[r + 1]);
                else acc = __builtin_elementwise_maximum(acc, h);
            } else if (rg == 0) {
                acc = __builtin_elementwise_maximum(acc, h);
            }
            diag = H[r];
            H[r] = h;
            up = h;
          }
        };
        auto col_done = [&](const V up, const V f, const int jj) {
            if constexpr (kSh && F16) {
                dl_h[jj] = P::bits(up + dsh_h);
                if constexpr (AFFINE) dl_f[jj] = P::bits(f + dsh_h);
            } else {
                dl_h[jj] = P::bits(up);
                if constexpr (AFFINE) dl_f[jj] = P::bits(f);
            }
        };
        auto col_start = [&](V& up, V& diag, V& f, const int jj) {
            const uint32_t u = (AFFINE || jj % 2 == 0) ? lo_lo(bin[jj], dl_h[jj]) : hi_lo(bin[jj], dl_h[jj]);
            up = P::from(u);
            if constexpr (F16 && !AFFINE) up = up - grp_h;
            diag = P::from(dtop);
            dtop = u;
            if constexpr (AFFINE) f = P::from(hi_lo(bin[jj], dl_f[jj]));
            if constexpr (F16) f = f - grp_h;
        };
        V up = P::from(0u), diag = P::from(0u), f = P::from(0u);
#pragma unroll
        for (int t = 0; t < STEPS; ++t) {
            const int jj = t / NCH;
            const int k = t % NCH;
            const uint32_t dep = P::bits(k == 0 ? H[R - 1] : H[CR * k - 1]);
            if (t + 1 < STEPS) {
                const int jn = (t + 1) / NCH, kn = (t + 1) % NCH;
                if (kn == 0) {
                    aa = code_row<RB>(rc, jn, blo);
                    ab = code_row<RB>(rp, jn, bhi);
                }
                read_x2a<CQ>(PL[(t + 1) & 1], PH[(t + 1) & 1], aa, ab, kn, dep);
            } else if (has_next && !next_t1 && !next_t2) {
                aa = code_row<RB>(rn, 0, blo);
                ab = code_row<RB>(rc, 0, bhi);
                read_x2a<CQ>(PL[(t + 1) & 1], PH[(t + 1) & 1], aa, ab, 0, dep);
            }
            if (k == 0) col_start(up, diag, f, jj);
            const int4(&pl)[CQ] = PL[t & 1];
            const int4(&ph)[CQ] = PH[t & 1];
            const int n = RL - CR * k < CR ? (RL - CR * k > 0 ? RL - CR * k : 0) : CR;
            if constexpr (F16 && AFFINE) {
                V dd[CR];
#pragma unroll
                for (int i = 0; i < CR; ++i)
                    if (i < n)
                        dd[i] = __builtin_elementwise_fma(P::from(word(pl, i)), P::from(word(ph, i)),
                                                          i == 0 ? diag : H[CR * k + i - 1]);
#pragma unroll
                for (int i = 0; i < CR; ++i)
                    if (i < n) asm volatile("" : "+v"(dd[i]));
#pragma unroll
                for (int i = 0; i < CR; ++i)
                    if (i < n) cell_d(CR * k + i, jj, up, diag, f, dd[i]);
            } else {
#pragma unroll
                for (int i = 0; i < CR; ++i)
                    if (i < n) cell(CR * k + i, jj, up, diag, f, P::from(word(pl, i)), P::from(word(ph, i)));
            }
            if (k == NCH - 1) col_done(up, f, jj);
            if constexpr (!F16) asm volatile("" : "+v"(best.v));
            else best.pin();
            __builtin_amdgcn_sched_barrier(0);
        }
        const bool high_last = CHAIN ? chain_last && (lo_c == 0 ? lo_p : lo_p + 1) >= npass : last;
        if (!high_last && col0 >= SG) {
            uint32_t hb[SG];
#pragma unroll
            for (int q = 0; q < SG; ++q) hb[q] = AFFINE ? hi_hi(dl_h[q], dl_f[q]) : hi_hi(dl_h[q], dl_h[q]);
            const uint32_t pc = CHAIN ? (lo_c == 0 ? ncols - SG : lo_c - SG) : col0 - SG;
            if (PAIR && ring_out) {
                if constexpr (kPairFlags) {
                    const int x = static_cast<int>(pc / SG);
                    pair_wait(ps->prog, ps->succ, x >= kRingSlots ? ps->base + x - kRingSlots + 1 : ps->base - 2);
                }
                ring_store<SG>(ring_out, (pc / SG) % kRingSlots, lane, hb);
            } else {
                const uint64_t poff = (pc >> 4) * kGroupBytes + (pc & 15);
                store_bnd<SG, AFFINE>(bnd, base + poff, hb);
            }
        }
        if (has_next) {
#pragma unroll
            for (int q = 0; q < SG / 4; ++q) {
                rp[q] = rc[q];
                rc[q] = rn[q];
            }
#pragma unroll
            for (int q = 0; q < SG; ++q) bin[q] = (next_first || !next_lo) ? bz[q] : bin_n[q];
        }
        if constexpr (PAIR && kPairFlags) {
            __builtin_amdgcn_fence(__ATOMIC_RELEASE, "workgroup");
            __hip_atomic_store(ps->prog + ps->me, ps->base + static_cast<int>(col0 / SG) + 1, __ATOMIC_RELAXED,
                               __HIP_MEMORY_SCOPE_WORKGROUP);
        } else if constexpr (PAIR) {
            __syncthreads();
            ++*tick;
        }
        if constexpr (CHAIN) {
            t2 = t1;
            lo_c = nreal;
            lo_p += wrap ? 1u : 0u;
        }
    }
}

__device__ __forceinline__ uint32_t block_cols(const InterArgs& a, int blk) {
    return a.blk_cols ? a.blk_cols[blk] : a.blk_groups[blk] * kGroupCols;
}

template <int R, int SG, bool AFFINE, bool F16, int CR, bool SHORT>
__device__ __forceinline__ bool x2s_block(const InterArgs& a, int blk, X2Lds<R>& L, int lane) {
    const uint32_t ncols = block_cols(a, blk);
    const uint64_t base = a.blk_off[blk] + static_cast<uint64_t>(lane) * kGroupCols;
    Best<F16> best;
    best.init(a);
    const uint64_t t0 = trace_now();
    const bool sh = SHORT && a.re_last == R - 4 && (ncols < 32 || ncols >= 64);
    const int full_end = a.qpad - (sh ? 2 * R : 0);
    const int chained = ncols >= 32 ? full_end / (2 * R) : 0;
    int s0 = 0;
    if (chained > 1) {
        x2s_pass<R, SG, AFFINE, F16, false, CR, true>(a, L, ncols, base, lane, 0, best, nullptr, nullptr, nullptr,
                                                      nullptr, chained);
        s0 = chained * 2 * R;
    }
    for (; s0 < full_end && ncols > 0; s0 += 2 * R)
        x2s_pass<R, SG, AFFINE, F16, false, CR>(a, L, ncols, base, lane, s0, best, nullptr, nullptr, nullptr);
    if constexpr (SHORT) {
        if (sh && ncols > 0)
            x2s_pass<R, SG, AFFINE, F16, false, CR, false, R - 4>(a, L, ncols, base, lane, full_end, best, nullptr,
                                                                  nullptr, nullptr);
    }
    const bool flagged = x2s_finish<F16>(a, blk, lane, best.value(a));
    trace_block(a, blk, t0, lane, 0);
    return flagged;
}

constexpr int kPairLag = 3;
constexpr int kPairCR = 8;
constexpr int kSingleCR = 8;
constexpr int kGroupWavesPerEU = 2;

__device__ __forceinline__ int group_ticks(uint32_t ncols, int passes, int SG, int G) {
    if (ncols == 0 || passes <= 0) return 0;
    const int S = static_cast<int>(ncols) / SG + 1;
    const int per = max(S, G * kPairLag);
    int t = 0;
    for (int p = max(0, passes - G); p < passes; ++p) t = max(t, (p / G) * per + kPairLag * (p % G) + S);
    return t;
}

template <int R, int SG, int GMAX>
struct X2pSmem {
    X2Lds<R> lds[kWavesPerWG];
    int4 ring[kWavesPerWG - kWavesPerWG / GMAX][kRingSlots * (SG / 4) * kLanes];
    uint32_t part[kWavesPerWG][kLanes];
    int prog[kWavesPerWG];
};

template <int R, int SG, bool AFFINE, bool F16, bool MERGED, int GMAX>
__device__ __forceinline__ bool x2p_wg(const InterArgs& a, int wgi, int quad_end, X2pSmem<R, SG, GMAX>& sm) {
    static_assert(R % 16 == 0 && SG % 4 == 0, "shape");
    static_assert(GMAX == 2 || GMAX == 4, "groups of 2 or 4 waves");
    X2Lds<R>* lds = sm.lds;
    auto& ring = sm.ring;
    auto& part = sm.part;
    using P = PkCell<F16>;
    using V = typename P::V;
    const int tid = tid_x();
    const int wave = __builtin_amdgcn_readfirstlane(tid >> 6);
    const int lane = tid & 63;
    const int npair = MERGED ? a.blk_first : a.nblocks;
    const int qend = GMAX == 4 ? quad_end : a.blk_base;
    const int qwg = qend - a.blk_base;
    const int pwg = qwg + (npair - qend + 1) / 2;
    const int tail = MERGED && a.blk_tail > npair && a.blk_tail < a.nblocks ? a.blk_tail : a.nblocks;
    const bool tri_on = MERGED && GMAX == 4 && AFFINE && a.blk_tri != 0;
    const int nspare = tri_on ? max(0, min(qwg, tail - npair)) : 0;
    const int s0 = npair + nspare;
    const int twg = pwg + (tail - s0 + kWavesPerWG - 1) / kWavesPerWG;
    const bool tailp = MERGED && wgi >= twg;
    const bool singles = MERGED && wgi >= pwg && !tailp;
    const bool quad = !tailp && wgi < qwg;
    const bool tri = tri_on && quad;
    const bool spare = tri && wave == kWavesPerWG - 1;
    const int G = tri ? 3 : quad ? 4 : 2, NG = tri ? 1 : kWavesPerWG / G;
    const int first = quad ? a.blk_base + wgi : tailp ? tail + (wgi - twg) * 2 : qend + (wgi - qwg) * 2;
    const int gend = tailp ? a.nblocks : npair;
    const int gi = spare ? 0 : wave / G, w = spare ? 0 : wave % G;
    const int passes = (a.qpad + 2 * R - 1) / (2 * R);
    int tmax = 0;
    for (int q = 0; q < NG; ++q) {
        const int b = first + q;
        if (b < gend) tmax = max(tmax, group_ticks(block_cols(a, b), passes, SG, G));
    }
    const int blk = first + gi;
    Best<F16> best;
    best.init(a);
    int tick = 0;
    const uint64_t t0 = trace_now();
    constexpr bool kPairFlags = pair_flags<AFFINE>();
    if constexpr (kPairFlags) {
        if (tid < kWavesPerWG) sm.prog[tid] = 0;
        __syncthreads();
    }
    bool flagged = false;
    const int sb = singles ? s0 + (wgi - pwg) * kWavesPerWG + wave : npair + wgi;
    if ((singles && sb < tail) || (spare && sb < s0))
        flagged = x2s_block<R, SG, AFFINE, F16, kSingleCR>(a, sb, lds[wave], lane);
    if (singles) return flagged;
    if (!spare && blk < gend) {
        const uint32_t ncols = block_cols(a, blk);
        const uint64_t base = a.blk_off[blk] + static_cast<uint64_t>(lane) * kGroupCols;
        const int per = max(static_cast<int>(ncols) / SG + 1, G * kPairLag);
        const int4* rin = w > 0 ? ring[gi * (G - 1) + w - 1] : nullptr;
        int4* rout = w < G - 1 ? ring[gi * (G - 1) + w] : nullptr;
        PairSync ps{sm.prog, wave, 0, -1, 0, w < G - 1 ? wave + 1 : -1, static_cast<int>(ncols) / SG + 1};
        auto enter = [&](const int p) {
            if constexpr (kPairFlags) {
                const int k = p / G;
                ps.base = k * ps.S;
                ps.pred = p == 0 ? -1 : w > 0 ? wave - 1 : wave + G - 1;
                ps.pred_base = (w > 0 ? k : k - 1) * ps.S;
            } else {
                const int start = (p / G) * per + kPairLag * w;
                while (tick < start) {
                    __syncthreads();
                    ++tick;
                }
            }
        };
        const int pfull = passes - (a.re_last == R - 4 ? 1 : 0);
        int p = w;
        for (; p < pfull && ncols > 0; p += G) {
            enter(p);
            x2s_pass<R, SG, AFFINE, F16, true, kPairCR>(a, lds[wave], ncols, base, lane, p * 2 * R, best, rin, rout,
                                                        &tick, &ps);
        }
        if (p == pfull && pfull < passes && ncols > 0) {
            enter(p);
            x2s_pass<R, SG, AFFINE, F16, true, kPairCR, false, R - 4>(a, lds[wave], ncols, base, lane, p * 2 * R, best,
                                                                      rin, rout, &tick, &ps);
        }
    }
    (void)tmax;
    if constexpr (!kPairFlags) {
        while (tick < tmax) {
            __syncthreads();
            ++tick;
        }
    }
    if (!spare && blk < gend && w > 0) part[wave][lane] = P::bits(best.value(a));
    __syncthreads();
    if (!spare && blk < gend && w == 0) {
        V b = best.value(a);
        for (int u = 1; u < G; ++u) {
            const V o = P::from(part[wave + u][lane]);
            if constexpr (F16) b = __builtin_elementwise_maximum(b, o);
            else b = max2(b, o);
        }
        flagged = x2s_finish<F16>(a, blk, lane, b);
        trace_block(a, blk, t0, lane, tri ? 3 : quad ? 4 : 1);
    }
    return flagged;
}

template <int R, int SG, bool AFFINE, bool F16, bool MERGED, int G>
__global__ __launch_bounds__(256, kGroupWavesPerEU) void sw_inter_x2p(InterArgs a) {
    __shared__ __attribute__((aligned(16))) X2pSmem<R, SG, G> sm;
    x2p_wg<R, SG, AFFINE, F16, MERGED, G>(a, blockIdx.x, MERGED ? a.blk_first : a.nblocks, sm);
}


template <bool AFFINE>
struct DrainShape {
    static constexpr int R16 = AFFINE ? 32 : 48, SG16 = AFFINE ? 8 : 4;
    static constexpr int R32 = AFFINE ? 32 : 64;
};
template <bool AFFINE, int RI>
constexpr size_t drain_smem() {
    using D = DrainShape<AFFINE>;
    const size_t x16 = kWavesPerWG * sizeof(X2Lds<D::R16>);
    const size_t i32 = static_cast<size_t>(kProfileRows) * intra_stride(RI);
    const size_t a32 = static_cast<size_t>(kWavesPerWG) * kProfileRows * inter_stride(D::R32);
    const size_t i16 = sizeof(typename ix2::IntraImg<RI, false>::Elem) * ix2::img_elems<RI, false>();
    return std::max(std::max(x16, i32), std::max(a32, i16));
}

template <bool AFFINE, int RI>
__device__ __forceinline__ void lpt_drain(const DrainArgs* __restrict__ d, char* smem, int* task) {
    using D = DrainShape<AFFINE>;
    for (;;) {
        const int tid = tid_x();
        const int wave = __builtin_amdgcn_readfirstlane(tid >> 6);
        const int lane = tid & 63;
        __syncthreads();
        if (tid == 0) {
            constexpr int kOrder[4] = {2, 0, 3, 1};
            constexpr int kWant[4] = {2 * kWavesPerWG, kWavesPerWG, 1, kWavesPerWG};
            int kind = 0, n = 0, start = 0;
            for (int k = 0; k < 4 && !n; ++k) {
                const int l = kOrder[k];
                if ((n = list_claim(d->lists[l], d->heads[l], kWant[k], &start))) kind = l + 1;
            }
            int m = 0;
            for (int i = 0; i < n; ++i) {
                const int v = list_wait_take(d->lists[kind - 1] + 1, start + i, d->fault, d->spin);
                if (v >= 0) task[2 + m++] = v;
            }
            task[0] = m ? kind : (n ? -1 : 0);
            task[1] = m;
        }
        __syncthreads();
        const int kind = task[0], n = task[1];
        if (kind == 0) return;
        if (kind < 0) continue;
        __builtin_amdgcn_fence(__ATOMIC_ACQUIRE, "agent");
        if (kind == 3) {
            IntraArgs y = d->i16;
            y.subj_list = task + 2;
            y.list_count = task + 1;
            ix2::intra_x2_wg<RI, false, true, !AFFINE, false, false, false, true>(y, 0,
                                                               reinterpret_cast<typename ix2::IntraImg<RI, false>::Elem*>(smem));
        } else if (kind == 1) {
            if (wave < n)
                x2s_block<D::R16, D::SG16, AFFINE, false, 16, false>(d->a16, task[2 + wave],
                                                              reinterpret_cast<X2Lds<D::R16>*>(smem)[wave], lane);
        } else if (kind == 4) {
            if (wave == 0) intra_subject<RI, AFFINE, false>(d->i32, task[2], reinterpret_cast<uint8_t*>(smem));
        } else {
            if (wave < n)
                inter_block<D::R32, 8, AFFINE, false>(
                    d->a32, task[2 + wave],
                    reinterpret_cast<uint8_t*>(smem) + wave * (kProfileRows * inter_stride(D::R32)), lane);
        }
    }
}

struct LptParams {
    InterArgs a;
    IntraArgs ia;
    const int32_t* order;
    const DrainArgs* drain;
    int32_t* next;
    int32_t n;
    int32_t grid;
};

template <int R, int SG, bool AFFINE, int RI, bool LOOP>
__global__ __launch_bounds__(256, kGroupWavesPerEU) void sw_scan_lpt(LptParams prm) {
    using Elem = typename ix2::IntraImg<RI, true>::Elem;
    using PElem = typename ix2::IntraImg<2, true>::Elem;
    constexpr size_t kInter = sizeof(X2pSmem<R, SG, 4>);
    constexpr size_t kIntra = sizeof(Elem) * ix2::img_elems<RI, true>();
    constexpr size_t kPipe = kWavesPerWG * sizeof(PElem) * ix2::img_elems<2, true>() + kWavesPerWG * sizeof(int);
    constexpr size_t kDrain = drain_smem<AFFINE, RI>();
    constexpr size_t kSmem = std::max(std::max(std::max(kInter, kIntra), kDrain), kPipe);
    __shared__ __attribute__((aligned(16))) char smem[kSmem];
    __shared__ int task[2 + 2 * kWavesPerWG];
    __shared__ int claimed;
    if (static_cast<int>(blockIdx.x) >= prm.n) return;
    for (int k = blockIdx.x;;) {
        auto kp = __builtin_amdgcn_kernarg_segment_ptr();
        if constexpr (LOOP) asm volatile("" : "+s"(kp));
        const LptParams& p = *(const LptParams*)(kp);
        const InterArgs& a = p.a;
        const IntraArgs& ia = p.ia;
        const int niwg = ((ia.nsubj + 1) / 2 + kWavesPerWG - 1) / kWavesPerWG;
        const int item = p.order[k];
        const uint64_t t0 = trace_now();
        bool flagged;
        if (item >= 0)
            flagged = x2p_wg<R, SG, AFFINE, true, true, 4>(a, item, a.blk_quad,
                                                           *reinterpret_cast<X2pSmem<R, SG, 4>*>(smem));
        else if (-1 - item < niwg)
            flagged = ix2::intra_x2_wg<RI, true, false, !AFFINE, true, false, AFFINE, true>(
                ia, -1 - item, reinterpret_cast<Elem*>(smem));
        else
            flagged = ix2::intra_x2_wg<2, true, false, !AFFINE, true, true, AFFINE, true>(
                ia, -1 - item - niwg, reinterpret_cast<PElem*>(smem));
        const int tw = tid_x();
        const bool wany = __builtin_amdgcn_ballot_w64(flagged) != 0;
        if ((tw & 63) == 0) task[2 + (tw >> 6)] = wany;
        __syncthreads();
        const bool any = (task[2] | task[3] | task[4] | task[5]) != 0;
        if (threadIdx.x == 0) trace_block(a, a.nblocks + k, t0, 0, item >= 0 ? 2 : 3);
        if (p.drain && any) lpt_drain<AFFINE, RI>(p.drain, smem, task);
        if constexpr (!LOOP) break;
        if (threadIdx.x == 0) claimed = p.grid + __hip_atomic_fetch_add(p.next, 1, __ATOMIC_RELAXED, __HIP_MEMORY_SCOPE_AGENT);
        __syncthreads();
        k = claimed;
        __syncthreads();
        if (k >= p.n) break;
    }
}

template <int R, int RI, bool AFFINE>
static int lpt_slots(int cus) {
    static const int per = [] {
        int p = 0;
        if (hipOccupancyMaxActiveBlocksPerMultiprocessor(&p, sw_scan_lpt<R, 8, AFFINE, RI, true>,
                                                         kWavesPerWG * kLanes, 0) != hipSuccess)
            return 0;
        return p;
    }();
    return cus * per;
}

constexpr int kLptLoopRounds = 3;

template <int R, int RI, bool AFFINE>
static void launch_lpt_t(const InterArgs& a, const IntraArgs& ia, const int32_t* order, int n, int cus,
                         hipStream_t s, const DrainArgs* drain, int32_t* next, int loop_grid) {
    int slots = next ? lpt_slots<R, RI, AFFINE>(cus) : 0;
    const dim3 block(kWavesPerWG * kLanes);
    if (next && loop_grid > 0) slots = std::min(loop_grid, n);
    if (slots > 0 && (n >= kLptLoopRounds * slots || (next && loop_grid > 0))) {
        const LptParams p{a, ia, order, drain, next, n, slots};
        hipLaunchKernelGGL((sw_scan_lpt<R, 8, AFFINE, RI, true>), dim3(slots), block, 0, s, p);
    } else {
        const LptParams p{a, ia, order, drain, nullptr, n, n};
        hipLaunchKernelGGL((sw_scan_lpt<R, 8, AFFINE, RI, false>), dim3(n), block, 0, s, p);
// ... 72 lines not shown
```

ece1782-smith-waterman-cuda_amd/csrc/sw_kernels.h:

```cpp
#pragma once

#include <hip/hip_runtime.h>
#include <stdint.h>

#include <string>

#include "sw_amd.h"

namespace swk {

int set_error(int code, const std::string& msg);

constexpr int kLanes = 64;
constexpr int kGroupCols = 16;
constexpr int kGroupBytes = kLanes * kGroupCols;
constexpr int kProfileRows = 32;
constexpr int kPadCode = 25;
constexpr uint8_t kStored[26] = {11, 1, 5, 2, 22, 6, 14, 12, 23, 9, 10, 0, 24, 7, 4, 15, 3, 21, 8, 13, 16, 17, 18, 19, 20, 25};
constexpr uint8_t kCodeOf[26] = {11, 1, 3, 16, 14, 2, 5, 13, 18, 9, 10, 0, 7, 19, 6, 15, 20, 21, 22, 23, 24, 17, 4, 8, 12, 25};
constexpr int kWavesPerWG = 4;
constexpr int kIntraSteps = 40;

template <int SG>
struct Residues {
    uint32_t w[SG / 4];
    __device__ __forceinline__ void load(const uint8_t* p) {
        if constexpr (SG == 16) {
            const int4 v = *reinterpret_cast<const int4*>(p);
            w[0] = v.x; w[1] = v.y; w[2] = v.z; w[3] = v.w;
        } else if constexpr (SG == 8) {
            const int2 v = *reinterpret_cast<const int2*>(p);
            w[0] = v.x; w[1] = v.y;
        } else {
            w[0] = *reinterpret_cast<const uint32_t*>(p);
        }
    }
    __device__ __forceinline__ uint32_t code(int jj) const { return (w[jj >> 2] >> (8 * (jj & 3))) & 0xffu; }
};

struct InterArgs {
    const uint8_t* residues;
    const uint64_t* blk_off;
    const uint32_t* blk_groups;
    const uint32_t* blk_cols;
    const int32_t* lane_ids;
    int32_t nblocks;
    const int8_t* prof;
    int32_t prof_stride;
    int32_t qpad;
    int32_t gap_open;
    int32_t gap_extend;
    int32_t* bnd_h;
    int32_t* bnd_f;
    int32_t* scores;
    int32_t* rescue_list;
    int32_t* rescue_count;
    const int32_t* blk_list;
    const int32_t* blk_count;
    int32_t blk_first;
    int32_t sat_limit;
    uint32_t f16_step[32];
    uint32_t f16_gog;
    uint32_t f16_zero;
    uint32_t f16_diff[3];
    int32_t blk_base;
    int32_t blk_quad;
    int32_t blk_tri;
    int32_t blk_tail;
    int32_t* rescue_max;
    uint64_t* trace;
    int32_t re_last;
};

struct IntraArgs {
    const uint8_t* residues;
    const uint64_t* subj_off;
    const int32_t* subj_len;
    const int32_t* subj_id;
    int32_t nsubj;
    const int8_t* prof;
    int32_t qpad;
    int32_t gap_open;
    int32_t gap_extend;
    int32_t* bnd_h;
    int32_t* bnd_f;
    int32_t* scores;
    int32_t prof_stride = 0;
    int32_t bias = 0;
    int32_t sat_limit = 0;
    uint32_t f16_step[kIntraSteps] = {};
    uint32_t f16_zero = 0;
    uint32_t f16_gog = 0;
    int32_t* rescue_list = nullptr;
    int32_t* rescue_count = nullptr;
    const int32_t* subj_list = nullptr;
    const int32_t* list_count = nullptr;
    int32_t pipe_pairs = 0;
    int32_t pipe_tail = 0x7fffffff;
};

#if defined(__HIPCC__)
__device__ __forceinline__ int tid_x() {
    int t = static_cast<int>(threadIdx.x);
    asm volatile("" : "+v"(t));
    return t;
}
__device__ __forceinline__ void list_publish(int32_t* items, int32_t* count, int32_t item) {
    __threadfence();
    const int slot = atomicAdd(count, 1);
    __hip_atomic_store(items + slot, item, __ATOMIC_RELAXED, __HIP_MEMORY_SCOPE_AGENT);
}
__device__ __forceinline__ int32_t list_take(const int32_t* items, int i) {
    int32_t* p = const_cast<int32_t*>(items) + i;
    const int32_t v = __builtin_amdgcn_readfirstlane(__hip_atomic_load(p, __ATOMIC_RELAXED, __HIP_MEMORY_SCOPE_AGENT));
    __hip_atomic_store(p, -1, __ATOMIC_RELAXED, __HIP_MEMORY_SCOPE_AGENT);
    return v;
}
__device__ __forceinline__ int32_t list_wait_take(int32_t* items, int i, int32_t* fault, int32_t bound) {
    int32_t* p = items + i;
    int32_t v = -1;
    for (int spin = 0; spin < bound; ++spin) {
        v = __hip_atomic_load(p, __ATOMIC_RELAXED, __HIP_MEMORY_SCOPE_AGENT);
        if (v >= 0) break;
        __builtin_amdgcn_s_sleep(1);
    }
    if (v >= 0)
        __hip_atomic_store(p, -1, __ATOMIC_RELAXED, __HIP_MEMORY_SCOPE_AGENT);
    else if (fault)
        __hip_atomic_store(fault, 1, __ATOMIC_RELAXED, __HIP_MEMORY_SCOPE_SYSTEM);
    return v;
}
__device__ __forceinline__ int list_claim(int32_t* count, int32_t* head, int want, int* start) {
    int h = __hip_atomic_load(head, __ATOMIC_RELAXED, __HIP_MEMORY_SCOPE_AGENT);
    for (int tries = 0; tries < 256; ++tries) {
        const int c = __hip_atomic_load(count, __ATOMIC_RELAXED, __HIP_MEMORY_SCOPE_AGENT);
        if (h >= c) return 0;
        const int nh = h + want < c ? h + want : c;
        if (__hip_atomic_compare_exchange_strong(head, &h, nh, __ATOMIC_RELAXED, __ATOMIC_RELAXED,
                                                 __HIP_MEMORY_SCOPE_AGENT)) {
            *start = h;
            return nh - h;
        }
    }
    return 0;
}
#endif

struct InterShape {
    int R, SG;
    bool x2s = false;
    bool f16 = false;
};
inline bool inter_needs_rescue(const InterShape& v, int x2_ok) { return v.f16 || (v.x2s && x2_ok != 2); }
inline bool inter_has_pair(const InterShape& v) { return v.x2s && v.R == 64 && v.SG == 8; }
inline int inter_coop_divisor(const InterShape& v) { return v.x2s ? 0 : 530000; }
int intra_chunk_bytes(int ri);
__host__ __device__ constexpr int intra_rip(int RI) { return (RI + 3) / 4 * 4; }

hipError_t launch_inter(const InterArgs& a, bool affine, const InterShape& v, hipStream_t s);
constexpr int kCoopRows = 32;
hipError_t launch_inter_coop(const InterArgs& a, int ncoop, bool affine, bool skew, hipStream_t s);
hipError_t launch_inter_x2s(const InterArgs& a, int R, int SG, bool affine, bool f16, hipStream_t s);
hipError_t launch_inter_x2s_list(const InterArgs& a, bool affine, hipStream_t s);
hipError_t launch_inter_x2p(const InterArgs& a, bool affine, bool f16, bool merged, int group, hipStream_t s);
struct DrainArgs {
    InterArgs a16;
    InterArgs a32;
    IntraArgs i16;
    IntraArgs i32;
    int32_t* lists[4];
    int32_t* heads[4];
    int32_t* fault;
    int32_t spin;
};
hipError_t launch_scan_lpt(const InterArgs& a, const IntraArgs& ia, const int32_t* order, int n, bool affine, int ri, int cus,
                           hipStream_t s, const DrainArgs* drain = nullptr, int32_t* next = nullptr,
                           int loop_grid = 0, int rows = 64);
constexpr int kSat16 = 32767 - 1152;
constexpr int kIntraX2MaxRI = 20;
constexpr int intra_period(int ri) { return ri == kIntraX2MaxRI ? 16 : 8; }
constexpr int intra_bias_rows(int ri) { return ri + intra_period(ri) + 2 > 26 ? ri + intra_period(ri) + 2 : 26; }

hipError_t launch_inter_rescue(const InterArgs& a, bool affine, hipStream_t s);
hipError_t launch_intra(const IntraArgs& a, int ri, bool affine, hipStream_t s);
hipError_t launch_intra_x2(const IntraArgs& a, int ri, hipStream_t s);
hipError_t launch_intra_x2_list16(const IntraArgs& a, int ri, hipStream_t s);
hipError_t launch_intra_x2_int16(const IntraArgs& a, int ri, hipStream_t s);

struct AlignArgs {
    const uint8_t* query;
    int32_t qlen;
    const uint8_t* subj;
    const int64_t* subj_off;
    int32_t n;
    const int8_t* mat;
    const int8_t* pssm = nullptr;
    int32_t pssm_ld = 0;
    int32_t gap;
    int32_t gap_extend;
    uint8_t* dirs;
    const int64_t* dirs_off;
    int32_t* hbuf;
    int32_t* out;
    char* ops;
    int64_t ops_stride;
};
hipError_t launch_align(const AlignArgs& a, hipStream_t s);

struct SynthFill {
    uint8_t* res;
    const uint64_t* blk_off;
    const uint32_t* blk_groups;
    const int32_t* lane_local;
    const int32_t* lane_len;
    int64_t nblocks;
    uint8_t* lres;
    const uint64_t* loff;
// ... 53 lines not shown
```

ece1782-smith-waterman-cuda_amd/csrc/sw_plan.cpp:

```cpp
#include "sw_plan.h"

#include <algorithm>
#include <cmath>
#include <cstdio>
#include <utility>
#include <vector>

namespace swplan {

namespace {
int32_t round_up(int64_t v, int64_t m) { return static_cast<int32_t>((v + m - 1) / m * m); }
}


constexpr int64_t kSmallDbSubjects = 64 * 1000;

constexpr double kFillSubjects = 570000.0;

int32_t default_long_threshold(const PlanDb& db) {
    if (db.n == 0) return 1536;
    const double mean = static_cast<double>(db.residues) / static_cast<double>(db.n);
    if (db.n < kSmallDbSubjects && mean >= 256) return 64;
    const double fill = db.n < kSmallDbSubjects ? 1.0 : std::min(1.0, static_cast<double>(db.n) / kFillSubjects);
    const double t = 5.7 * mean * std::pow(fill, 0.4);
// ... 98 lines not shown
    const int64_t swg = (tail - s0 + swk::kWavesPerWG - 1) / swk::kWavesPerWG;
    const int64_t twg = (nb - tail + 1) / 2;
    const int64_t npairs = (db.nlong + 1) / 2;
    const int64_t iwg = (npairs + swk::kWavesPerWG - 1) / swk::kWavesPerWG;
    const int nch = qpad_intra / (swk::kLanes * ri);
    const double step_us = intra_step_us(ri);
    std::vector<std::pair<double, int32_t>> w;
    w.reserve(static_cast<size_t>(pwg + swg + twg + iwg));
    auto width = [&](int64_t b) { return static_cast<int64_t>(db.blk_groups[b]) * swk::kGroupCols; };
    for (int64_t g = 0; g < nquad; ++g) {
        double c = group_ticks_host(width(g), passes, tri ? 3 : 4);
        if (g < nspare) c = std::max(c, single_ticks(width(npair + g), passes));
        w.emplace_back(c * tick_us, g);
    }
    for (int64_t g = nquad; g < pwg; ++g) {
        double c = 0;
        for (int q = 0; q < 2; ++q) {
            const int64_t b = nquad + (g - nquad) * 2 + q;
            if (b < npair) c = std::max(c, group_ticks_host(width(b), passes, 2));
        }
        w.emplace_back(c * tick_us, static_cast<int32_t>(g));
    }
    for (int64_t g = 0; g < swg; ++g)
        w.emplace_back(single_ticks(width(s0 + g * swk::kWavesPerWG), passes) * tick_us,
                       static_cast<int32_t>(pwg + g));
    for (int64_t g = 0; g < twg; ++g) {
        w.emplace_back(group_ticks_host(width(tail + 2 * g), passes, 2) * tick_us,
                       static_cast<int32_t>(pwg + swg + g));
    }
    const int nchp = (qpad_intra + 127) / 128;
    double inter_max = 0;
    for (const auto& e : w) inter_max = std::max(inter_max, e.first);
    auto pair_us = [&](int64_t p) { return (db.llen[static_cast<size_t>(2 * p)] + swk::kLanes - 1) * nch *
                                           step_us; };
    int64_t npipe = 0;
    if (nchp <= swk::kWavesPerWG) {
        if (db.opts->lpt_pipe >= 0) npipe = db.opts->lpt_pipe;
        else
            while (npipe < std::min<int64_t>(npairs, 4) && pair_us(npipe) > inter_max) ++npipe;
    }
    npipe = std::min(npipe, npairs);
    int64_t ntp = 0;
    if (db.opts->lpt_pipe_tail >= 0) ntp = db.opts->lpt_pipe_tail;
    else if (!affine && static_cast<double>(db.n) < kQuadMaxFill * kFillSubjects) ntp = (npairs * 2 / 100 + 4) / 8 * 8;
    if (nchp > swk::kWavesPerWG) ntp = 0;
    ntp = std::max<int64_t>(0, std::min(ntp, npairs - npipe));
    const int64_t pipe_tail = npairs - ntp;
    const int64_t npipe_wg = npipe / swk::kWavesPerWG;
    for (int64_t g = npipe_wg; g < iwg; ++g) {
        const int64_t first = std::max<int64_t>(8 * g, 2 * npipe);
        if (first >= db.nlong || first >= 2 * pipe_tail) continue;
        w.emplace_back((db.llen[static_cast<size_t>(first)] + swk::kLanes - 1) * nch * step_us,
                       static_cast<int32_t>(-1 - g));
    }
    for (int64_t p = 0; p < npipe; ++p) w.emplace_back(1e30 - p, static_cast<int32_t>(-1 - (iwg + p)));
    const double pstep_us = intra_step_us(2);
    for (int64_t p = pipe_tail; p < npairs; ++p)
        w.emplace_back((db.llen[static_cast<size_t>(2 * p)] + swk::kLanes - 1 + 128.0 * (nchp - 1)) * pstep_us,
                       static_cast<int32_t>(-1 - (iwg + p)));
    std::stable_sort(w.begin(), w.end(), [](const std::pair<double, int32_t>& x, const std::pair<double, int32_t>& y) {
        return x.first > y.first;
    });
    LptPlan out;
    out.order.resize(w.size());
    out.cost.resize(w.size());
    for (size_t k = 0; k < w.size(); ++k) {
        out.order[k] = w[k].second;
        out.cost[k] = static_cast<float>(w[k].first);
    }
    out.npipe = static_cast<int32_t>(npipe);
    out.pipe_tail = static_cast<int32_t>(pipe_tail);
    return out;
}

swk::InterShape inter_shape(bool affine, int x2_ok, const sw_opts& o) {
    using swk::InterShape;
    const bool y_ok = x2_ok == 2 || (x2_ok == 1 && o.int16_guard != 0);
    InterShape v = y_ok ? InterShape{64, 8, true, true} : InterShape{affine ? 32 : 64, 8};
    if (const char* e = o.inter_variant; e[0]) {
        int r = 0, g = 0;
        if (std::sscanf(e, "f%dx%d", &r, &g) == 2 && y_ok && r == 32 && (g == 8 || (g == 4 && affine)))
            v = InterShape{2 * r, g, true, true};
        else if (std::sscanf(e, "y%dx%d", &r, &g) == 2 && y_ok && r == 32 && g == 8)
            v = InterShape{2 * r, g, true, false};
        else if (std::sscanf(e, "%dx%d", &r, &g) == 2 && g == 8 && (r == 32 || r == 64))
            v = InterShape{r, g};
    }
    return v;
}

std::string inter_kernel_name(const swk::InterShape& v, bool affine) {
    char b[96];
    if (v.x2s)
        std::snprintf(b, sizeof b, "sw_inter_x2s<%d,%d,%s%s>", v.R / 2, v.SG, affine ? "affine" : "linear",
                      v.f16 ? ",fp16" : "");
    else
        std::snprintf(b, sizeof b, "sw_inter<%d,%d,%s>", v.R, v.SG, affine ? "affine" : "linear");
    return b;
}

int rescue_rows(bool affine) { return affine ? 32 : 64; }

int intra_rows_for(int qlen, int longest) {
    int best_ri = 16;
    double best_cost = 1e300;
    for (int ri = 2; ri <= 16; ri += 2) {
        const int chunk = swk::kLanes * ri;
        const int nch = (qlen + chunk - 1) / chunk;
        const double cost = static_cast<double>(nch) * (longest + swk::kLanes - 1) * (ri * 3.7 + 8.0);
        if (cost < best_cost) { best_cost = cost; best_ri = ri; }
    }
    return best_ri;
}

int intra_x2_rows_for(int qlen, int longest, int wide, int forced) {
    if (forced > 0) {
        const int ri = forced;
        if (ri == 4 || ri == 6 || ri == 8 || ri == 10 || ri == 12 || ri == 16) return ri;
        if (ri == swk::kIntraX2MaxRI && wide >= 1) return ri;
    }
    int best_ri = 16;
    double best_cost = 1e300;
    for (int ri : {4, 6, 8, 10, 12, 16, swk::kIntraX2MaxRI}) {
        if (ri == swk::kIntraX2MaxRI && wide < 2) continue;
        const int chunk = swk::kLanes * ri;
        const int nch = (qlen + chunk - 1) / chunk;
        const double cost = static_cast<double>(nch) * (longest + swk::kLanes - 1) * (ri * 28.8 + 80.0);
        if (cost < best_cost) {
            best_cost = cost;
            best_ri = ri;
        }
    }
    return best_ri;
}

bool lpt_supported(int ri) { return ri == 4 || ri == 6 || ri == 8; }

int32_t short_rows(int32_t qlen, int pass_rows) {
    const int32_t left = qlen - (round_up(qlen, pass_rows) / pass_rows - 1) * pass_rows;
    return (left + 1) / 2 <= pass_rows / 2 - 4 ? pass_rows / 2 - 4 : pass_rows / 2;
}

PlanScoring plan_scoring(const int8_t* m, int go, int ge) {
    PlanScoring s;
    s.go = go;
    s.ge = ge;
    for (int k = 0; k < 625; ++k) {
        s.max_s = std::max<int>(s.max_s, m[k]);
        if (m[k] + go > 127) s.biased_fits = false;
    }
    return s;
}

PlanScoring plan_scoring_max(int max_entry, int go, int ge) {
    PlanScoring s;
    s.go = go;
    s.ge = ge;
    s.max_s = std::max(0, max_entry);
    s.biased_fits = max_entry + go <= 127;
    return s;
}

PlanScoring plan_scoring_pssm(const int8_t* rows, int32_t qlen, int go, int ge) {
    int mx = -128;
    for (int64_t k = 0; k < static_cast<int64_t>(qlen) * 25; ++k) mx = std::max<int>(mx, rows[k]);
    return plan_scoring_max(mx, go, ge);
}

ScanPlan scan_plan(const PlanDb& db, int32_t qlen, const PlanScoring& s, bool intra_i16_first, int32_t i16_span) {
    const sw_opts& O = *db.opts;
    const int max_s = s.max_s, go = s.go, ge = s.ge;
    ScanPlan p;
    p.affine = go != ge || !s.biased_fits;
    const bool affine = p.affine;
    const bool f16_fits = 2 * max_s + 27 * ge + go < 1024;
    p.x2_ok = !f16_fits                                                   ? 0
              : (static_cast<int64_t>(qlen) + 2) * (max_s + go) < 32767 ? 2
              : (max_s + go < 1000 && ge < 1000)                       ? 1
                                                                       : 0;
    p.shape = inter_shape(affine, p.x2_ok, O);
    const int R = p.shape.R;
    p.rescue = swk::inter_needs_rescue(p.shape, p.x2_ok);
    p.f16 = p.shape.f16;
    p.qpad_rescue = p.rescue ? round_up(qlen, rescue_rows(affine)) : 0;
    const int list_rows = affine ? 64 : 96;
    p.qpad_list = p.f16 ? round_up(qlen, list_rows) : 0;

    p.intra_x2 = db.nlong && p.x2_ok >= 1 && O.intra_x2 != 0;
    p.intra_i16_first = intra_i16_first && p.intra_x2;
    const bool ri2_wide =
        db.nblocks == 0 && 2 * max_s + (swk::intra_bias_rows(swk::kIntraX2MaxRI) + 1) * ge + go < 1024;
    const int ri2_model =
        p.intra_x2 ? intra_x2_rows_for(qlen, db.long_max, ri2_wide ? (affine ? 2 : 1) : 0, O.intra_x2_rows) : 0;
    const int ri2_lpt = (affine && ri2_model > 8 && db.nblocks && O.intra_x2_rows < 0) ? 8 : ri2_model;

    p.npair = (db.nblocks && swk::inter_has_pair(p.shape) && round_up(qlen, R) > R) ? pair_blocks(db) : 0;
    p.ncoop = (!p.npair && db.nblocks) ? coop_blocks(db, swk::inter_coop_divisor(p.shape)) : 0;
    p.qpad_coop = p.ncoop ? round_up(qlen, swk::kCoopRows) : 0;
    p.nr = (p.f16 && p.rescue && p.npair && !p.ncoop) ? i16_span : 0;

    const bool lpt_want = O.lpt >= 0 ? O.lpt == 1 : true;
    p.lpt = lpt_want && db.nlong && db.nblocks && p.intra_x2 && !p.intra_i16_first && p.f16 && p.rescue &&
            p.npair && !p.ncoop && i16_span == 0 && lpt_supported(ri2_lpt);
    p.lpt_rows = (p.lpt && !affine && O.lpt_rows != 64 && round_up(qlen, 96) > 96) ? 96 : 64;
    p.qpad_inter = round_up(qlen, p.lpt_rows == 96 ? 96 : R);
    p.re_last = p.shape.x2s ? short_rows(qlen, p.lpt_rows == 96 ? 96 : R) : 0;
    if (p.lpt) {
        const int passes = p.qpad_inter / p.lpt_rows;
        p.ntri = affine ? lpt_tri_blocks(db, p.npair, passes) : 0;
        p.nquad = p.ntri ? p.ntri : lpt_quad_blocks(db, p.npair);
        p.ntail = lpt_tail_blocks(db, p.npair, passes);
    }

    p.ri = db.nlong ? intra_rows_for(qlen, db.long_max) : 0;
    p.qpad_intra = p.ri ? round_up(qlen, static_cast<int64_t>(swk::kLanes) * p.ri) : 0;
    p.ri2 = p.lpt ? ri2_lpt : ri2_model;
    p.qpad_intra2 = p.ri2 ? round_up(qlen, static_cast<int64_t>(swk::kLanes) * p.ri2) : 0;
    p.multi_inter = p.qpad_inter > R || p.qpad_rescue > rescue_rows(affine) || p.qpad_coop > swk::kCoopRows ||
                    p.qpad_list > list_rows;
    p.multi_intra = (p.ri && p.qpad_intra > swk::kLanes * p.ri) || (p.ri2 && p.qpad_intra2 > swk::kLanes * p.ri2);

    if (db.nblocks) {
        p.kernel = inter_kernel_name(p.shape, affine);
        if (p.npair) p.kernel.replace(0, sizeof("sw_inter_x2s") - 1, "sw_inter_x2p");
        if (p.lpt_rows == 96) p.kernel.replace(p.kernel.find("<32,"), 4, "<48,");
        if (p.nr) p.kernel += "+int16[0," + std::to_string(p.nr) + ")";
        if (p.ntail) p.kernel += "+tail" + std::to_string(p.ntail);
        if (p.ntri) p.kernel += "+tri" + std::to_string(p.ntri);
        if (p.lpt) p.kernel += "+lpt";
    }
    p.intra_kernel = !db.nlong   ? "none"
                     : p.intra_x2 ? "sw_intra_x2<" + std::to_string(p.ri2) + (p.intra_i16_first ? ",int16>" : ">")
                                  : "sw_intra<" + std::to_string(p.ri) + (affine ? ",affine>" : ",linear>");
    return p;
}

void ScanPlan::set_drain(bool got_rows) {
    if (!lpt || !got_rows || drain) return;
    drain = true;
    ri = ri2;
    qpad_intra = qpad_intra2;
    multi_intra = qpad_intra > swk::kLanes * ri;
    kernel += "+drain";
}

}
```

ece1782-smith-waterman-cuda_amd/csrc/sw_plan.h:

```cpp
#pragma once

#include <cstdint>
#include <string>
#include <vector>

#include "sw_amd.h"
#include "sw_kernels.h"

namespace swplan {

struct PlanDb {
    int64_t n = 0;
    int64_t residues = 0;
    int64_t nblocks = 0;
    int64_t nlong = 0;
    int32_t long_threshold = 0;
    int32_t long_max = 0;
    const uint32_t* blk_groups = nullptr;
    const int32_t* llen = nullptr;
    const sw_opts* opts = nullptr;
    int cus = 0;
};

int32_t default_long_threshold(const PlanDb& db);
int32_t coop_blocks(const PlanDb& db, int divisor);
int pair_group(const PlanDb& db);
int32_t pair_blocks(const PlanDb& db);
int32_t lpt_quad_blocks(const PlanDb& db, int32_t npair);
int32_t lpt_tri_blocks(const PlanDb& db, int32_t npair, int passes);
int32_t lpt_tail_blocks(const PlanDb& db, int32_t npair, int passes);
double intra_step_us(int ri);
double single_ticks(int64_t ncols, int passes);
double group_ticks_host(int64_t ncols, int passes, int G);

swk::InterShape inter_shape(bool affine, int x2_ok, const sw_opts& o);
std::string inter_kernel_name(const swk::InterShape& v, bool affine);
int rescue_rows(bool affine);
int intra_rows_for(int qlen, int longest);
int intra_x2_rows_for(int qlen, int longest, int wide, int forced);
bool lpt_supported(int ri);
int32_t short_rows(int32_t qlen, int pass_rows);

struct PlanScoring {
    int max_s = 0;
    int go = 0, ge = 0;
    bool biased_fits = true;
};
PlanScoring plan_scoring(const int8_t* matrix625, int go, int ge);
PlanScoring plan_scoring_pssm(const int8_t* rows, int32_t qlen, int go, int ge);
PlanScoring plan_scoring_max(int max_entry, int go, int ge);

struct ScanPlan {
    bool affine = false;
    int x2_ok = 0;
    swk::InterShape shape{};
    bool rescue = false;
    bool f16 = false;
    bool intra_x2 = false;
    bool intra_i16_first = false;
    int ri = 0;
    int ri2 = 0;
    int32_t qpad_inter = 0, qpad_intra = 0, qpad_intra2 = 0, qpad_rescue = 0, qpad_list = 0, qpad_coop = 0;
    int32_t npair = 0;
    int32_t ncoop = 0;
    int32_t nr = 0;
    bool lpt = false;
    bool drain = false;
    int lpt_rows = 64;
    int32_t re_last = 0;
    int32_t ntri = 0, nquad = 0, ntail = 0;
    bool multi_inter = false, multi_intra = false;
    std::string kernel, intra_kernel;

    void set_drain(bool got_rows);
};

ScanPlan scan_plan(const PlanDb& db, int32_t qlen, const PlanScoring& s, bool intra_i16_first, int32_t i16_span);

struct LptPlan {
    std::vector<int32_t> order;
    std::vector<float> cost;
    int32_t npipe = 0;
    int32_t pipe_tail = 0;
};
LptPlan lpt_plan(const PlanDb& db, int32_t qpad, int rows, int32_t qpad_intra, int ri, int32_t npair, int32_t nquad,
                 int32_t ntail, bool affine, bool tri);

}
```

include/sw_amd.h:

```cpp
#ifndef SW_AMD_H
#define SW_AMD_H

#include <stdint.h>

#ifdef __cplusplus
extern "C" {
#endif

#if defined(SW_AMD_BUILD)
#define SW_API __attribute__((visibility("default")))
#else
#define SW_API
#endif

#define SW_OK 0
#define SW_E_INVALID -1
#define SW_E_HIP -2
#define SW_E_NOMEM -3
#define SW_E_NODEVICE -4
#define SW_E_UNSUPPORTED -5
#define SW_E_IO -6
#define SW_E_DEVICE -7

#define SW_ALPHABET 25
#define SW_CODE_STAR 24

#define SW_MATRIX_BLOSUM50_REF 0
#define SW_MATRIX_BLOSUM62 1
#define SW_MATRIX_IDENTITY3 2
#define SW_MATRIX_BLOSUM50_CHAR 3

typedef struct sw_scoring {
    const int8_t* matrix;
    int32_t gap_open;
    int32_t gap_extend;
} sw_scoring;

typedef struct sw_db_stats {
    int64_t n_subjects;
    int64_t residues;
    int64_t packed_cells;
    int64_t n_blocks;
    int64_t n_long;
    int64_t device_bytes;
    int32_t max_length;
    int32_t long_threshold;
    int32_t coop_blocks;
    int64_t coop_residues;
    int32_t max_id;
    int32_t pair_blocks;
    int32_t pair_merged;
    int64_t pair_residues;
} sw_db_stats;

typedef struct sw_timing {
    float inter_ms;
    float intra_ms;
    float total_ms;
    int32_t rescued;
    int32_t launches;
    float coop_ms;
    float wave_ms;
} sw_timing;

typedef struct sw_handle sw_handle;
typedef struct sw_db sw_db;

SW_API int32_t sw_version(void);
SW_API const char* sw_build_id(void);
SW_API const char* sw_last_error(void);
SW_API int sw_encode(const char* ascii, int64_t n, uint8_t* codes);
SW_API int sw_builtin_matrix(int32_t id, int8_t* out625);

SW_API int sw_create(int32_t device, sw_handle** out);
SW_API int sw_destroy(sw_handle* h);
SW_API void* sw_stream(sw_handle* h);
SW_API int sw_set_stream(sw_handle* h, void* hip_stream);

typedef struct sw_opts {
    int32_t size;
    int32_t lpt;
    int32_t lpt_pipe;
    int32_t quad_width;
    int32_t pair_width;
    int32_t pair_group;
    int32_t coop_width;
    int32_t coop_skew;
    int32_t intra_x2;
    int32_t intra_x2_rows;
    int32_t intra_i16_first;
    int32_t inter_i16_span;
    int32_t int16_guard;
    int32_t rescue_stats;
    int32_t tail_pairs;
    int32_t lpt_persist;
    int32_t lpt_rows;
    int32_t tri_width;
    int32_t lpt_pipe_tail;
    int32_t drain_spin;
    char inter_variant[16];
    char trace_file[256];
} sw_opts;
SW_API int sw_opts_init(sw_opts* o);
SW_API int sw_opts_from_env(sw_opts* o);
SW_API int sw_set_opts(sw_handle* h, const sw_opts* o);
SW_API int sw_get_opts(const sw_handle* h, sw_opts* o);

SW_API int sw_db_create(sw_handle* h, const uint8_t* residues, const int64_t* offsets,
                 int64_t n, const int32_t* ids, sw_db** out);
SW_API int sw_db_free(sw_db* db);
SW_API int sw_db_get_stats(const sw_db* db, sw_db_stats* out);
SW_API int sw_db_save(const sw_db* db, const char* path);
SW_API int sw_db_load(sw_handle* h, const char* path, sw_db** out);
SW_API int sw_db_create_synthetic(sw_handle* h, uint64_t seed, int64_t id_base, int64_t n,
                                  sw_db** out);
SW_API int sw_synth_tables(int32_t* len4096, uint8_t* lut65536);
SW_API int sw_synth_lengths(uint64_t seed, int64_t id_base, int64_t n, int32_t* lengths);
SW_API int sw_db_subjects(const sw_db* db, int64_t* lengths, int32_t* ids);
SW_API int sw_db_set_long_threshold(sw_db* db, int32_t threshold);
SW_API int sw_db_reset_adaptive(sw_db* db);

SW_API int sw_scan(sw_handle* h, const sw_db* db, const uint8_t* query, int32_t qlen,
            const sw_scoring* sc, int32_t* scores_host);

SW_API int sw_scan_device(sw_handle* h, const sw_db* db, const uint8_t* query, int32_t qlen,
                   const sw_scoring* sc, int32_t* scores_dev);

SW_API int sw_scan_batch(sw_handle* h, const sw_db* db, const uint8_t* queries,
                  const int64_t* qoffsets, int32_t nq, const sw_scoring* sc,
                  int32_t* scores_host);
SW_API int sw_scan_batch_device(sw_handle* h, const sw_db* db, const uint8_t* queries,
                  const int64_t* qoffsets, int32_t nq, const sw_scoring* sc,
                  int32_t* scores_dev);

SW_API int sw_get_timing(sw_handle* h, sw_timing* out);
SW_API int sw_timing_reset(sw_handle* h);
SW_API int sw_timing_total(sw_handle* h, sw_timing* out, int32_t* nscans);
SW_API int sw_stream_wait_scan(sw_handle* h, void* hip_stream);
SW_API const char* sw_last_kernel(sw_handle* h);
SW_API const char* sw_last_intra_kernel(sw_handle* h);

SW_API int sw_topk(const int32_t* scores, int64_t n, int32_t k, int32_t* out_ids,
            int32_t* out_scores);

SW_API int sw_topk_device(sw_handle* h, const int32_t* scores_dev, int64_t n, int64_t id_base,
                   int32_t k, int64_t* keys_out_dev);
SW_API int sw_topk_keys_device(sw_handle* h, const int64_t* keys_dev, int64_t n, int32_t k,
                        int64_t* keys_out_dev);
SW_API int sw_scan_topk(sw_handle* h, const sw_db* db, const uint8_t* query, int32_t qlen,
                        const sw_scoring* sc, int32_t k, int64_t* keys_host);
SW_API int sw_topk_device_ids(sw_handle* h, const int32_t* scores_dev, int64_t n, const int32_t* ids_dev,
                              int32_t k, int64_t* keys_out_dev);
SW_API int sw_scan_rank_device(sw_handle* h, const sw_db* db, const uint8_t* query, int32_t qlen,
                               const sw_scoring* sc, int32_t* scores_dev, int32_t k, const int32_t* gid_dev,
                               int64_t id_base, int64_t* keys_out_dev);

typedef struct sw_alignment {
    int32_t score;
    int32_t q_begin, q_end;
    int32_t s_begin, s_end;
    int32_t ops_len;
} sw_alignment;
SW_API int sw_align(sw_handle* h, const sw_db* db, const uint8_t* query, int32_t qlen,
                    const sw_scoring* sc, const int32_t* ids, int32_t n, sw_alignment* out,
                    char* ops, int64_t ops_stride);

typedef struct sw_pssm sw_pssm;
SW_API int sw_pssm_create(sw_handle* h, const int8_t* rows, int32_t qlen, sw_pssm** out);
SW_API int sw_pssm_free(sw_pssm* p);
SW_API int sw_pssm_length(const sw_pssm* p, int32_t* qlen);
SW_API int sw_scan_pssm(sw_handle* h, const sw_db* db, const sw_pssm* p, int32_t gap_open,
                        int32_t gap_extend, int32_t* scores_host);
SW_API int sw_scan_pssm_device(sw_handle* h, const sw_db* db, const sw_pssm* p, int32_t gap_open,
                               int32_t gap_extend, int32_t* scores_dev);
SW_API int sw_scan_pssm_topk(sw_handle* h, const sw_db* db, const sw_pssm* p, int32_t gap_open,
                             int32_t gap_extend, int32_t k, int64_t* keys_host);
SW_API int sw_align_pssm(sw_handle* h, const sw_db* db, const sw_pssm* p, int32_t gap_open,
                         int32_t gap_extend, const int32_t* ids, int32_t n, sw_alignment* out,
                         char* ops, int64_t ops_stride);

SW_API int sw_score_pair(sw_handle* h, const uint8_t* query, int32_t qlen,
                  const uint8_t* subject, int32_t slen, const sw_scoring* sc,
                  int32_t* score);

typedef struct sw_group sw_group;
typedef struct sw_gdb sw_gdb;
SW_API int sw_group_create(const int32_t* devices, int32_t ndev, sw_group** out);
SW_API int sw_group_destroy(sw_group* g);
SW_API const char* sw_group_info(const sw_group* g);
SW_API int sw_group_handle(sw_group* g, int32_t d, sw_handle** out);
SW_API int sw_group_db_create(sw_group* g, const uint8_t* residues, const int64_t* offsets, int64_t n,
                              const int32_t* ids, sw_gdb** out);
SW_API int sw_group_db_free(sw_gdb* gdb);
SW_API int sw_group_db_shard(const sw_gdb* gdb, int32_t d, int64_t* n_subjects, int64_t* residues);
SW_API int sw_group_scan(sw_group* g, const sw_gdb* gdb, const uint8_t* query, int32_t qlen,
                         const sw_scoring* sc, int32_t* scores_host);
SW_API int sw_group_topk(sw_group* g, const sw_gdb* gdb, const uint8_t* query, int32_t qlen,
                         const sw_scoring* sc, int32_t k, int64_t* keys_host);

#ifdef __cplusplus
}
#endif
#endif
```

Before: 11310.

## Amortize f16 rebias via periodic drift table in affine SG=8 inter kernel

Replaces the per-column-group subtraction of the rebias constant on all H/E registers with a lazily accumulated drift. Per-row offsets come from a precomputed bias table, and the drift is subtracted from the state only every few columns or at pass boundaries, while only the accumulators and boundary constants are adjusted each step. This removes many packed f16 subtracts from the inner loop, at the cost of less saturation headroom (handled by drift_rows gating), a much larger InterArgs kernarg struct, and extra template instantiations. Kernels also read their arguments through the kernarg segment pointer instead of a by-value copy.

```diff
diff --git a/ece1782-smith-waterman-cuda_amd/capi.py b/ece1782-smith-waterman-cuda_amd/capi.py
--- a/ece1782-smith-waterman-cuda_amd/capi.py
+++ b/ece1782-smith-waterman-cuda_amd/capi.py
@@ -18,7 +18,7 @@
 EXPORTED = (
     "sw_version", "sw_build_id", "sw_last_error", "sw_encode", "sw_builtin_matrix",
     "sw_create", "sw_destroy", "sw_stream", "sw_set_stream",
-    "sw_opts_init", "sw_opts_from_env", "sw_set_opts", "sw_get_opts",
+    "sw_opts_init", "sw_opts_from_env", "sw_set_opts", "sw_get_opts", "sw_f16_bias",
     "sw_db_create", "sw_db_free", "sw_db_get_stats", "sw_db_set_long_threshold", "sw_db_reset_adaptive",
     "sw_scan", "sw_scan_device", "sw_scan_batch", "sw_scan_batch_device", "sw_get_timing",
     "sw_timing_reset", "sw_timing_total", "sw_stream_wait_scan", "sw_last_kernel", "sw_last_intra_kernel",
@@ -62,14 +62,27 @@
     INT_FIELDS = ("lpt", "lpt_pipe", "quad_width", "pair_width", "pair_group", "coop_width", "coop_skew",
                   "intra_x2", "intra_x2_rows", "intra_i16_first", "inter_i16_span", "int16_guard",
                   "rescue_stats", "tail_pairs", "lpt_persist", "lpt_rows", "tri_width", "lpt_pipe_tail", "drain_spin")
+    TAIL_INT_FIELDS = ("bias_period",)
     _fields_ = [("size", ctypes.c_int32)] + [(f, ctypes.c_int32) for f in INT_FIELDS] + \
-        [("inter_variant", ctypes.c_char * 16), ("trace_file", ctypes.c_char * 256)]
+        [("inter_variant", ctypes.c_char * 16), ("trace_file", ctypes.c_char * 256)] + \
+        [(f, ctypes.c_int32) for f in TAIL_INT_FIELDS]
 
     def as_dict(self):
-        d = {f: getattr(self, f) for f in self.INT_FIELDS}
+        d = {f: getattr(self, f) for f in self.INT_FIELDS + self.TAIL_INT_FIELDS}
         d["inter_variant"] = self.inter_variant.decode()
         d["trace_file"] = self.trace_file.decode()
         return d
+
+
+F16_BIAS_TABLE = 536
+
+
+def f16_bias(max_s, gap_extend, bias_period=-1):
+    period, sat, rows = ctypes.c_int32(), ctypes.c_int32(), ctypes.c_int32()
+    tbl = np.zeros(F16_BIAS_TABLE, dtype=np.uint32)
+    _check(lib().sw_f16_bias(int(max_s), int(gap_extend), int(bias_period), ctypes.byref(period), ctypes.byref(sat),
+                             ctypes.byref(rows), tbl.ctypes.data_as(ctypes.POINTER(ctypes.c_uint32)), tbl.size))
+    return period.value, sat.value, tbl, rows.value
 
 
 def opts_from_env():
@@ -118,6 +131,7 @@
         "sw_opts_from_env": (ctypes.c_int, [ctypes.POINTER(Opts)]),
         "sw_set_opts": (ctypes.c_int, [vp, ctypes.POINTER(Opts)]),
         "sw_get_opts": (ctypes.c_int, [vp, ctypes.POINTER(Opts)]),
+        "sw_f16_bias": (ctypes.c_int, [i32, i32, i32, i32p, i32p, i32p, ctypes.POINTER(ctypes.c_uint32), i32]),
         "sw_db_reset_adaptive": (ctypes.c_int, [vp]),
         "sw_db_create": (ctypes.c_int, [vp, u8p, i64p, i64, i32p, ctypes.POINTER(vp)]),
         "sw_db_free": (ctypes.c_int, [vp]),
@@ -254,7 +268,7 @@
         for k, v in fields.items():
             if k in ("inter_variant", "trace_file"):
                 setattr(o, k, (v or "").encode())
-            elif k in Opts.INT_FIELDS:
+            elif k in Opts.INT_FIELDS or k in Opts.TAIL_INT_FIELDS:
                 setattr(o, k, -1 if v is None else int(v))
             else:
                 raise TypeError("unknown sw_opts field %r" % k)
diff --git a/ece1782-smith-waterman-cuda_amd/csrc/sw_capi.cpp b/ece1782-smith-waterman-cuda_amd/csrc/sw_capi.cpp
--- a/ece1782-smith-waterman-cuda_amd/csrc/sw_capi.cpp
+++ b/ece1782-smith-waterman-cuda_amd/csrc/sw_capi.cpp
@@ -31,6 +31,19 @@
     uint16_t b;
     std::memcpy(&b, &x, 2);
     return static_cast<uint32_t>(b) | (static_cast<uint32_t>(b) << 16);
+}
+
+static_assert(SW_F16_BIAS_TABLE == swk::kF16Tbl, "sw_amd.h states the table's size");
+int f16_bias_consts(int max_s, int ge, int period, uint32_t* tbl, int32_t* drift_rows) {
+    const int zero = -kF16Span + 2 * ge;
+    const int last = 8 * std::max(period, 1) + 24;
+    for (int i = 0; tbl && i < swk::kF16Tbl; ++i) {
+        const int j = std::min(i, last) - 1;
+        tbl[i] = (f16_pair((j + 8) * ge + zero) & 0xffffu) | (f16_pair(j * ge + zero) & 0xffff0000u);
+    }
+    const int sat = kF16Span - zero - 2 * std::max(max_s, 1) - 26 * ge;
+    if (drift_rows) *drift_rows = period > 0 ? std::max(0, sat - 8 * period * ge) / std::max(max_s, 1) : 0;
+    return sat;
 }
 
 int fail(int code, const std::string& msg) {
@@ -193,7 +206,7 @@
     for (int32_t* f : {&o.lpt, &o.lpt_pipe, &o.quad_width, &o.pair_width, &o.pair_group, &o.coop_width,
                        &o.coop_skew, &o.intra_x2, &o.intra_x2_rows, &o.intra_i16_first, &o.inter_i16_span,
                        &o.int16_guard, &o.rescue_stats, &o.tail_pairs, &o.lpt_persist, &o.lpt_rows,
-                       &o.tri_width, &o.lpt_pipe_tail, &o.drain_spin})
+                       &o.tri_width, &o.lpt_pipe_tail, &o.drain_spin, &o.bias_period})
         *f = -1;
     return o;
 }
@@ -1192,7 +1205,8 @@
         a.rescue_list = c.listA + 1;
         if (p.f16) a.rescue_max = c.maxA;
         const int zero = -kF16Span + 2 * ge;
-        a.sat_limit = kF16Span - zero - 2 * std::max(c.sc.max_s, 1) - 26 * ge;
+        a.f16_period = std::max<int>(p.bias_period, 1);
+        a.sat_limit = f16_bias_consts(c.sc.max_s, ge, p.bias_period, a.f16_tbl, &a.f16_drift_rows);
         for (int j = 0; j < 32; ++j) a.f16_step[j] = f16_pair(j * ge + zero);
         a.f16_gog = f16_pair(go - ge);
         a.f16_zero = f16_pair(zero);
@@ -1781,12 +1795,22 @@
                 {"SW_LPT_ROWS", &o->lpt_rows},
                 {"SW_TRI_WIDTH", &o->tri_width},
                 {"SW_LPT_PIPE_TAIL", &o->lpt_pipe_tail},
-                {"SW_DRAIN_SPIN", &o->drain_spin}};
+                {"SW_DRAIN_SPIN", &o->drain_spin},
+                {"SW_BIAS_PERIOD", &o->bias_period}};
     for (const auto& k : ints)
         if (const char* e = std::getenv(k.name); e && e[0]) *k.field = std::atoi(e);
     if (const char* e = std::getenv("SW_INTER_VARIANT"))
         std::snprintf(o->inter_variant, sizeof o->inter_variant, "%s", e);
     if (const char* e = std::getenv("SW_TRACE_FILE")) std::snprintf(o->trace_file, sizeof o->trace_file, "%s", e);
+    return SW_OK;
+}
+
+int sw_f16_bias(int32_t max_s, int32_t gap_extend, int32_t bias_period, int32_t* period, int32_t* sat_limit,
+                int32_t* drift_rows, uint32_t* table, int32_t table_len) {
+    if (!period || !sat_limit || !drift_rows || gap_extend < 0 || (table && table_len < swk::kF16Tbl))
+        return fail(SW_E_INVALID, "sw_f16_bias: null output, negative extend or a table under SW_F16_BIAS_TABLE entries");
+    *period = swplan::bias_period_for(gap_extend, bias_period);
+    *sat_limit = f16_bias_consts(max_s, gap_extend, *period, table, drift_rows);
     return SW_OK;
 }
 
diff --git a/ece1782-smith-waterman-cuda_amd/csrc/sw_inter_x2.hip b/ece1782-smith-waterman-cuda_amd/csrc/sw_inter_x2.hip
--- a/ece1782-smith-waterman-cuda_amd/csrc/sw_inter_x2.hip
+++ b/ece1782-smith-waterman-cuda_amd/csrc/sw_inter_x2.hip
@@ -210,9 +210,14 @@
 template <int R, int SG, bool AFFINE, bool F16, int CR = 16, bool SHORT = true>
 __device__ __forceinline__ bool x2s_block(const InterArgs& a, int blk, X2Lds<R>& L, int lane);
 
+__device__ __forceinline__ const InterArgs& kernarg_inter() {
+    return *(const InterArgs*)(__builtin_amdgcn_kernarg_segment_ptr());
+}
+
 template <int R, int SG, bool AFFINE, bool F16, bool LIST, int CR = 16>
-__global__ __launch_bounds__(256, 2) void sw_inter_x2s(InterArgs a) {
+__global__ __launch_bounds__(256, 2) void sw_inter_x2s(InterArgs) {
     static_assert(R % CR == 0 && SG % 4 == 0, "shape");
+    const InterArgs& a = kernarg_inter();
     __shared__ __attribute__((aligned(16))) X2Lds<R> lds[kWavesPerWG];
     const int wave = __builtin_amdgcn_readfirstlane(threadIdx.x >> 6);
     const int lane = threadIdx.x & 63;
@@ -346,10 +351,12 @@
         __builtin_amdgcn_s_sleep(1);
 }
 
-template <int R, int SG, bool AFFINE, bool F16, bool PAIR, int CR = 16, bool CHAIN = false, int RL = R>
+template <int R, int SG, bool AFFINE, bool F16, bool PAIR, int CR = 16, bool CHAIN = false, int RL = R,
+          bool DRIFT = false>
 __device__ __forceinline__ void x2s_pass(const InterArgs& a, X2Lds<R>& L, uint32_t ncols, uint64_t base, int lane,
                                          int s0, Best<F16>& best, const int4* ring_in, int4* ring_out,
-                                         int* tick, const PairSync* ps = nullptr, int chain_passes = 1) {
+                                         int* tick, const PairSync* ps = nullptr, int chain_passes = 1,
+                                         bool out_drift = false) {
     static_assert(!(CHAIN && PAIR), "chained passes: single-wave blocks only");
     constexpr int CQ = CR / 4;
     constexpr int NCH = R / CR;
@@ -368,6 +375,12 @@
         reb_h = __builtin_bit_cast(h2, a.f16_diff[SG == 4 ? 0 : 1]);
         grp_h = __builtin_bit_cast(h2, a.f16_diff[2]);
     }
+    constexpr bool kDrift = F16 && AFFINE && SG == 8 && DRIFT;
+    auto tbl = [&](const uint32_t n8, const int j) { return a.f16_tbl[n8 + j + 1]; };
+    auto drift_of = [&](const uint32_t n) {
+        return __builtin_bit_cast(h2, a.f16_tbl[8 * n + 1]) - __builtin_bit_cast(h2, a.f16_tbl[1]);
+    };
+    const uint32_t Q = kDrift ? static_cast<uint32_t>(a.f16_period) : 1u;
     const bool first = (s0 == 0);
     const bool last = (s0 + 2 * R >= a.qpad);
     const uint32_t npass = CHAIN ? static_cast<uint32_t>(chain_passes) : 1u;
@@ -375,7 +388,7 @@
     const uint32_t total = npass * ncols;
     const int sbias = F16 ? (AFFINE ? 2 : 1) * a.gap_extend : 0;
     const int gbias0 = F16 ? -kRowGroup * a.gap_extend : 0;
-    const uint32_t dtop0 = F16 ? a.f16_step[SG - 2 + kRowGroup] : 0u;
+    const uint32_t dtop0 = kDrift ? tbl(0, kRowGroup - 2) : F16 ? a.f16_step[SG - 2 + kRowGroup] : 0u;
     constexpr bool kSh = RL < R;
     if constexpr (kSh) asm volatile("" : "+v"(lane));
     static_assert(!kSh || (RL == R - 4 && !CHAIN), "rows per strip: R, or R - 4 outside a chain");
@@ -390,7 +403,8 @@
     V H[R];
     V E[AFFINE ? R : 1];
 #pragma unroll
-    for (int r = 0; r < R; ++r) H[r] = P::from(F16 ? a.f16_step[r % kRowGroup + SG - 1] : 0u);
+    for (int r = 0; r < R; ++r)
+        H[r] = P::from(kDrift ? tbl(0, r % kRowGroup - 1) : F16 ? a.f16_step[r % kRowGroup + SG - 1] : 0u);
 #pragma unroll
     for (int r = 0; r < (AFFINE ? R : 1); ++r) E[r] = P::from(F16 ? a.f16_zero : 0u);
     uint32_t dtop = dtop0;
@@ -401,6 +415,7 @@
 #pragma unroll
     for (int q = 0; q < SG; ++q) {
         bz[q] = !F16 ? 0u
+                     : kDrift ? lo_lo(tbl(0, kRowGroup - 1 + q), tbl(0, kRowGroup + q))
                      : AFFINE ? lo_lo(a.f16_step[kRowGroup - 1 + q], a.f16_step[kRowGroup + q])
                               : lo_lo(a.f16_step[kRowGroup - 1 + q], a.f16_step[kRowGroup - 1 + q]);
         dl_h[q] = F16 ? a.f16_step[kRowGroup - 1 + q] : 0u;
@@ -429,6 +444,15 @@
 
     uint32_t lo_p = 0, lo_c = 0;
     bool t2 = false;
+    uint32_t n = 0, jst = 0;
+    uint32_t fl[kAcc + 1] = {};
+    if constexpr (kDrift) {
+#pragma unroll
+        for (int j = 1; j <= kAcc; ++j) fl[j] = tbl(0, j);
+        const h2 lo8 = __builtin_bit_cast(h2, a.f16_diff[1] & 0xffffu);
+#pragma unroll
+        for (int k = 0; k < kAcc; ++k) best.acc[k] = best.acc[k] + lo8;
+    }
     for (uint32_t col0 = 0; col0 <= total; col0 += SG) {
         const bool has_next = col0 + SG <= total;
         const bool next_lo = col0 + SG < total;
@@ -444,7 +468,10 @@
             stage_x2s<R, F16>(L, prof16, a.prof_stride, static_cast<int>(lo_p) * 2 * R, lane, sbias, gbias0, 0);
 #pragma unroll
             for (int r = 0; r < R; ++r) {
-                H[r] = P::from(__builtin_amdgcn_perm(P::bits(H[r]), F16 ? a.f16_step[r % kRowGroup + SG - 1] : 0u,
+                H[r] = P::from(__builtin_amdgcn_perm(P::bits(H[r]),
+                                                     kDrift ? tbl(0, r % kRowGroup - 1)
+                                                     : F16  ? a.f16_step[r % kRowGroup + SG - 1]
+                                                            : 0u,
                                                      0x07060100u));
                 if constexpr (AFFINE) E[r] = P::from(__builtin_amdgcn_perm(P::bits(E[r]), F16 ? a.f16_zero : 0u, 0x07060100u));
             }
@@ -454,11 +481,13 @@
             stage_x2s<R, F16>(L, prof16, a.prof_stride, static_cast<int>(lo_p) * 2 * R, lane, sbias, gbias0, 1);
 #pragma unroll
             for (int r = 0; r < R; ++r) {
-                H[r] = P::from(__builtin_amdgcn_perm(F16 ? a.f16_step[r % kRowGroup + SG - 1] : 0u, P::bits(H[r]),
-                                                     0x07060100u));
+                H[r] = P::from(__builtin_amdgcn_perm(kDrift ? tbl(8 * n, r % kRowGroup - 1)
+                                                     : F16  ? a.f16_step[r % kRowGroup + SG - 1]
+                                                            : 0u,
+                                                     P::bits(H[r]), 0x07060100u));
                 if constexpr (AFFINE) E[r] = P::from(__builtin_amdgcn_perm(F16 ? a.f16_zero : 0u, P::bits(E[r]), 0x07060100u));
             }
-            dtop = __builtin_amdgcn_perm(dtop0, dtop, 0x07060100u);
+            dtop = __builtin_amdgcn_perm(kDrift ? tbl(8 * n, kRowGroup - 2) : dtop0, dtop, 0x07060100u);
         }
         if (t1 || t2) {
             __builtin_amdgcn_fence(__ATOMIC_RELEASE, "workgroup");
@@ -480,7 +509,7 @@
                 else load_bnd<SG, AFFINE>(bin_n, bnd, base + noff);
             }
         }
-        if constexpr (F16) {
+        if constexpr (F16 && !kDrift) {
 #pragma unroll
             for (int r = 0; r < R; ++r) {
                 if (r <= RL) H[r] = H[r] - reb_h;
@@ -529,7 +558,7 @@
             const h2 h = max3h(E[r], f, d);
             const h2 m = h - gog_h;
             E[r] = __builtin_elementwise_maximum(E[r], m);
-            f = max3h(f, m, __builtin_bit_cast(h2, a.f16_step[rg + jj + 1]));
+            f = max3h(f, m, __builtin_bit_cast(h2, kDrift ? fl[rg + jj + 1] : a.f16_step[rg + jj + 1]));
             h2& acc = best.acc[rg + jj];
             if (jj & 1) {
                 if (rg + 1 < kRowGroup) acc = max3h(acc, h, H[r + 1]);
@@ -610,6 +639,17 @@
             uint32_t hb[SG];
 #pragma unroll
             for (int q = 0; q < SG; ++q) hb[q] = AFFINE ? hi_hi(dl_h[q], dl_f[q]) : hi_hi(dl_h[q], dl_h[q]);
+            if constexpr (kDrift) {
+                const bool canon = !out_drift && (!CHAIN || (lo_c == 0 ? lo_p : lo_p + 1) >= npass);
+                if (canon) {
+                    const h2 d = drift_of(n);
+#pragma unroll
+                    for (int q = 0; q < SG; ++q) hb[q] = P::bits(P::from(hb[q]) - d);
+                } else if (jst) {
+#pragma unroll
+                    for (int q = 0; q < SG; ++q) hb[q] = P::bits(P::from(hb[q]) + P::from(jst));
+                }
+            }
             const uint32_t pc = CHAIN ? (lo_c == 0 ? ncols - SG : lo_c - SG) : col0 - SG;
             if (PAIR && ring_out) {
                 if constexpr (kPairFlags) {
@@ -622,6 +662,38 @@
                 store_bnd<SG, AFFINE>(bnd, base + poff, hb);
             }
         }
+        if constexpr (kDrift) {
+            if (has_next) {
+                const uint32_t jn = n + 1;
+                jst = 0;
+                uint32_t kd = P::bits(reb_h);
+                if (jn == Q || next_t1) {
+                    jst = __builtin_amdgcn_readfirstlane(P::bits(drift_of(jn)));
+                    const h2 J = P::from(jst);
+                    kd = __builtin_amdgcn_readfirstlane(P::bits(reb_h - J));
+#pragma unroll
+                    for (int r = 0; r < R; ++r) {
+                        if (r <= RL) H[r] = H[r] - J;
+                        if (r < RL) E[r] = E[r] - J;
+                    }
+                    dtop = P::bits(P::from(dtop) - J);
+#pragma unroll
+                    for (int q = 0; q < SG; ++q) {
+                        dl_h[q] = P::bits(P::from(dl_h[q]) - J);
+                        dl_f[q] = P::bits(P::from(dl_f[q]) - J);
+                    }
+                    n = 0;
+                } else {
+                    n = jn;
+                }
+#pragma unroll
+                for (int k = 0; k < kAcc; ++k) best.acc[k] = best.acc[k] + P::from(kd);
+#pragma unroll
+                for (int q = 0; q < SG; ++q) bz[q] = P::bits(P::from(bz[q]) + P::from(kd));
+#pragma unroll
+                for (int j = 1; j <= kAcc; ++j) fl[j] = tbl(8 * n, j);
+            }
+        }
         if (has_next) {
 #pragma unroll
             for (int q = 0; q < SG / 4; ++q) {
@@ -645,6 +717,27 @@
             lo_p += wrap ? 1u : 0u;
         }
     }
+    if constexpr (kDrift) {
+        const h2 d = drift_of(n) + __builtin_bit_cast(h2, a.f16_diff[1] & 0xffffu);
+#pragma unroll
+        for (int k = 0; k < kAcc; ++k) best.acc[k] = best.acc[k] - d;
+    }
+}
+
+template <int R, int SG, bool AFFINE, bool F16, bool PAIR, int CR, bool CHAIN, int RL>
+__device__ __forceinline__ void x2s_pass_any(const InterArgs& a, X2Lds<R>& L, uint32_t ncols, uint64_t base, int lane,
+                                             int s0, Best<F16>& best, const int4* ring_in, int4* ring_out, int* tick,
+                                             const PairSync* ps, int chain_passes, int rows_end) {
+    if constexpr (F16 && AFFINE && SG == 8) {
+        if (rows_end <= a.f16_drift_rows) {
+            x2s_pass<R, SG, AFFINE, F16, PAIR, CR, CHAIN, RL, true>(a, L, ncols, base, lane, s0, best, ring_in, ring_out,
+                                                                    tick, ps, chain_passes,
+                                                                    rows_end + 2 * R <= a.f16_drift_rows);
+            return;
+        }
+    }
+    x2s_pass<R, SG, AFFINE, F16, PAIR, CR, CHAIN, RL, false>(a, L, ncols, base, lane, s0, best, ring_in, ring_out, tick,
+                                                             ps, chain_passes);
 }
 
 __device__ __forceinline__ uint32_t block_cols(const InterArgs& a, int blk) {
@@ -663,16 +756,18 @@
     const int chained = ncols >= 32 ? full_end / (2 * R) : 0;
     int s0 = 0;
     if (chained > 1) {
-        x2s_pass<R, SG, AFFINE, F16, false, CR, true>(a, L, ncols, base, lane, 0, best, nullptr, nullptr, nullptr,
-                                                      nullptr, chained);
+        x2s_pass_any<R, SG, AFFINE, F16, false, CR, true, R>(a, L, ncols, base, lane, 0, best, nullptr, nullptr,
+                                                             nullptr, nullptr, chained, chained * 2 * R);
         s0 = chained * 2 * R;
     }
     for (; s0 < full_end && ncols > 0; s0 += 2 * R)
-        x2s_pass<R, SG, AFFINE, F16, false, CR>(a, L, ncols, base, lane, s0, best, nullptr, nullptr, nullptr);
+        x2s_pass_any<R, SG, AFFINE, F16, false, CR, false, R>(a, L, ncols, base, lane, s0, best, nullptr, nullptr,
+                                                              nullptr, nullptr, 1, s0 + 2 * R);
     if constexpr (SHORT) {
         if (sh && ncols > 0)
-            x2s_pass<R, SG, AFFINE, F16, false, CR, false, R - 4>(a, L, ncols, base, lane, full_end, best, nullptr,
-                                                                  nullptr, nullptr);
+            x2s_pass_any<R, SG, AFFINE, F16, false, CR, false, R - 4>(a, L, ncols, base, lane, full_end, best,
+                                                                      nullptr, nullptr, nullptr, nullptr, 1,
+                                                                      full_end + 2 * R);
     }
     const bool flagged = x2s_finish<F16>(a, blk, lane, best.value(a));
     trace_block(a, blk, t0, lane, 0);
@@ -777,13 +872,14 @@
         int p = w;
         for (; p < pfull && ncols > 0; p += G) {
             enter(p);
-            x2s_pass<R, SG, AFFINE, F16, true, kPairCR>(a, lds[wave], ncols, base, lane, p * 2 * R, best, rin, rout,
-                                                        &tick, &ps);
+            x2s_pass_any<R, SG, AFFINE, F16, true, kPairCR, false, R>(a, lds[wave], ncols, base, lane, p * 2 * R, best,
+                                                                      rin, rout, &tick, &ps, 1, (p + 1) * 2 * R);
         }
         if (p == pfull && pfull < passes && ncols > 0) {
             enter(p);
-            x2s_pass<R, SG, AFFINE, F16, true, kPairCR, false, R - 4>(a, lds[wave], ncols, base, lane, p * 2 * R, best,
-                                                                      rin, rout, &tick, &ps);
+            x2s_pass_any<R, SG, AFFINE, F16, true, kPairCR, false, R - 4>(a, lds[wave], ncols, base, lane, p * 2 * R,
+                                                                          best, rin, rout, &tick, &ps, 1,
+                                                                          (p + 1) * 2 * R);
         }
     }
     (void)tmax;
@@ -809,8 +905,9 @@
 }
 
 template <int R, int SG, bool AFFINE, bool F16, bool MERGED, int G>
-__global__ __launch_bounds__(256, kGroupWavesPerEU) void sw_inter_x2p(InterArgs a) {
+__global__ __launch_bounds__(256, kGroupWavesPerEU) void sw_inter_x2p(InterArgs) {
     __shared__ __attribute__((aligned(16))) X2pSmem<R, SG, G> sm;
+    const InterArgs& a = kernarg_inter();
     x2p_wg<R, SG, AFFINE, F16, MERGED, G>(a, blockIdx.x, MERGED ? a.blk_first : a.nblocks, sm);
 }
 
diff --git a/ece1782-smith-waterman-cuda_amd/csrc/sw_kernels.h b/ece1782-smith-waterman-cuda_amd/csrc/sw_kernels.h
--- a/ece1782-smith-waterman-cuda_amd/csrc/sw_kernels.h
+++ b/ece1782-smith-waterman-cuda_amd/csrc/sw_kernels.h
@@ -20,6 +20,13 @@
 constexpr uint8_t kCodeOf[26] = {11, 1, 3, 16, 14, 2, 5, 13, 18, 9, 10, 0, 7, 19, 6, 15, 20, 21, 22, 23, 24, 17, 4, 8, 12, 25};
 constexpr int kWavesPerWG = 4;
 constexpr int kIntraSteps = 40;
+constexpr int kF16PeriodMax = 64;
+constexpr int kF16DriftBudget = 512;
+constexpr int kF16Tbl = 8 * kF16PeriodMax + 24;
+__host__ __device__ constexpr int f16_period_for(int ge) {
+    const int q = ge > 0 ? kF16DriftBudget / (8 * ge) : kF16PeriodMax;
+    return q < 1 ? 1 : q > kF16PeriodMax ? kF16PeriodMax : q;
+}
 
 template <int SG>
 struct Residues {
@@ -63,6 +70,9 @@
     uint32_t f16_gog;
     uint32_t f16_zero;
     uint32_t f16_diff[3];
+    int32_t f16_period;
+    int32_t f16_drift_rows;
+    uint32_t f16_tbl[kF16Tbl];
     int32_t blk_base;
     int32_t blk_quad;
     int32_t blk_tri;
diff --git a/ece1782-smith-waterman-cuda_amd/csrc/sw_plan.cpp b/ece1782-smith-waterman-cuda_amd/csrc/sw_plan.cpp
--- a/ece1782-smith-waterman-cuda_amd/csrc/sw_plan.cpp
+++ b/ece1782-smith-waterman-cuda_amd/csrc/sw_plan.cpp
@@ -274,6 +274,11 @@
     return s;
 }
 
+int32_t bias_period_for(int ge, int forced) {
+    const int q = swk::f16_period_for(ge);
+    return forced >= 1 ? std::min(forced, q) : q;
+}
+
 PlanScoring plan_scoring_max(int max_entry, int go, int ge) {
     PlanScoring s;
     s.go = go;
@@ -327,6 +332,7 @@
     p.lpt_rows = (p.lpt && !affine && O.lpt_rows != 64 && round_up(qlen, 96) > 96) ? 96 : 64;
     p.qpad_inter = round_up(qlen, p.lpt_rows == 96 ? 96 : R);
     p.re_last = p.shape.x2s ? short_rows(qlen, p.lpt_rows == 96 ? 96 : R) : 0;
+    if (p.f16 && affine) p.bias_period = bias_period_for(ge, O.bias_period);
     if (p.lpt) {
         const int passes = p.qpad_inter / p.lpt_rows;
         p.ntri = affine ? lpt_tri_blocks(db, p.npair, passes) : 0;
diff --git a/ece1782-smith-waterman-cuda_amd/csrc/sw_plan.h b/ece1782-smith-waterman-cuda_amd/csrc/sw_plan.h
--- a/ece1782-smith-waterman-cuda_amd/csrc/sw_plan.h
+++ b/ece1782-smith-waterman-cuda_amd/csrc/sw_plan.h
@@ -40,6 +40,7 @@
 int intra_x2_rows_for(int qlen, int longest, int wide, int forced);
 bool lpt_supported(int ri);
 int32_t short_rows(int32_t qlen, int pass_rows);
+int32_t bias_period_for(int ge, int forced);
 
 struct PlanScoring {
     int max_s = 0;
@@ -68,6 +69,7 @@
     bool drain = false;
     int lpt_rows = 64;
     int32_t re_last = 0;
+    int32_t bias_period = 0;
     int32_t ntri = 0, nquad = 0, ntail = 0;
     bool multi_inter = false, multi_intra = false;
     std::string kernel, intra_kernel;
diff --git a/include/sw_amd.h b/include/sw_amd.h
--- a/include/sw_amd.h
+++ b/include/sw_amd.h
@@ -100,10 +100,14 @@
     int32_t drain_spin;
     char inter_variant[16];
     char trace_file[256];
+    int32_t bias_period;
 } sw_opts;
 SW_API int sw_opts_init(sw_opts* o);
 SW_API int sw_opts_from_env(sw_opts* o);
 SW_API int sw_set_opts(sw_handle* h, const sw_opts* o);
+#define SW_F16_BIAS_TABLE 536
+SW_API int sw_f16_bias(int32_t max_s, int32_t gap_extend, int32_t bias_period, int32_t* period,
+                       int32_t* sat_limit, int32_t* drift_rows, uint32_t* table, int32_t table_len);
 SW_API int sw_get_opts(const sw_handle* h, sw_opts* o);
 
 SW_API int sw_db_create(sw_handle* h, const uint8_t* residues, const int64_t* offsets,
```

Result: no change. 11360 (median of 6 runs) (+0.5%).
